# faverogian/diffusion-classifier

Measured on AMD Instinct MI355X. Metric: images classified/sec (node), CIFAR-10 10-class x 50-step ELBO scoring, higher is better.
Workload: dtype bf16; 1 GPU; cifar10-unet-10x50; classes=10, trials=50, forwards_per_image=500, input=uniform [-1,1], parallelism=single

## Files before the change

diffusion-classifier_amd/_lib.py:

```python
import ctypes as C
import os

_HERE = os.path.dirname(os.path.abspath(__file__))
LIB_PATH = os.environ.get("DCAMD_LIB") or os.path.join(_HERE, "libdcamd.so")

ABI_VERSION = 5
DC_F32, DC_BF16, DC_F16 = 0, 1, 2
ACT_NONE, ACT_SILU, ACT_GEGLU, ACT_GELU_TANH = 0, 1, 2, 3
OP_QSAMPLE, OP_SINUSOID, OP_IGEMM, OP_GROUPNORM, OP_LAYERNORM, OP_ATTENTION, OP_EPS_MSE, OP_TBLOCK_FRONT = 1, 2, 3, 4, 5, 6, 7, 8
OP_CROSS_ATTENTION = 9
OP_CROSS_ATTENTION_LEN = 10
OP_ATTENTION_BIAS, OP_RMSNORM, OP_EMBED_ROWS, OP_RELU = 11, 12, 13, 14
ATTENTION_BIAS_MAX_L = 512
OP_ATTENTION_CAUSAL, OP_LAYERNORM_ROWS, OP_EMBED_ROWS_POS, OP_ACT_PASS = 15, 16, 17, 18
ATTENTION_CAUSAL_MAX_L = 512
PASS_QUICK_GELU, PASS_GELU_ERF = 1, 2
OP_ERR_MAP = 19
EVIDENCE_FRAC_BITS, EVIDENCE_VMAX = 30, 16384.0
OP_ATTENTION_WIDE, OP_IM2COL_S2 = 20, 21
ATTENTION_WIDE_DIMS = (256, 512)

i32, i64, u64, f32, vp = C.c_int32, C.c_int64, C.c_uint64, C.c_float, C.c_void_p


class QsampleParams(C.Structure):
    _fields_ = [("x", vp), ("eps", vp), ("alpha", vp), ("sigma", vp), ("img_of_bj", vp),
                ("out", vp), ("out_dtype", i32),
                ("n_bj", i32), ("C", i32), ("H", i32), ("W", i32), ("ld", i32), ("im2col", i32), ("patch", i32)]


class SinusoidParams(C.Structure):
    _fields_ = [("lam", vp), ("out", vp), ("n", i32), ("dim", i32), ("flip_sin_to_cos", i32), ("freq_shift", f32)]


class IgemmParams(C.Structure):
    _fields_ = [("dtype", i32), ("taps", i32), ("stride", i32), ("upsample", i32),
                ("n_img", i32), ("Hin", i32), ("Win", i32), ("Hout", i32), ("Wout", i32),
                ("src0", vp), ("map0", vp), ("C0", i32), ("ld0", i32),
                ("src1", vp), ("map1", vp), ("C1", i32), ("ld1", i32),
                ("W", vp), ("Cout", i32), ("tile_n", i32),
                ("bias", vp),
                ("rowvec", vp), ("rowvec_map", vp), ("rowvec_ld", i32), ("act", i32),
                ("gate", vp), ("gate_map", vp), ("gate_ld", i32), ("pad2_", i32),
                ("residual", vp), ("res_map", vp), ("res_dtype", i32), ("res_ld", i32),
                ("out", vp), ("out_dtype", i32), ("out_ld", i32),
                ("gn_scale", vp), ("gn_shift", vp), ("gn_silu", i32), ("pad3_", i32),
                ("src2", vp), ("map2", vp), ("W2", vp), ("C2", i32), ("ld2", i32),
                ("ln_eps", f32), ("up4", i32), ("qstats", vp),
                ("pn_out", vp), ("pn_gamma", vp), ("pn_beta", vp), ("pn_cnt", vp),
                ("pn_ld", i32), ("pn_groups", i32), ("pn_silu", i32), ("pn_eps", f32)]


class GroupnormParams(C.Structure):
    _fields_ = [("x", vp), ("map0", vp), ("x1", vp), ("map1", vp),
                ("y", vp), ("dtype", i32), ("out_dtype", i32),
                ("n", i32), ("HW", i32), ("C", i32), ("C1", i32), ("groups", i32), ("silu", i32),
                ("splits", i32), ("eps", f32),
                ("gamma", vp), ("beta", vp), ("ws", vp), ("out_scale", vp), ("out_shift", vp),
                ("qstats", vp), ("qparts", i32), ("pad_", i32)]


class LayernormParams(C.Structure):
    _fields_ = [("x", vp), ("y", vp), ("dtype", i32), ("out_dtype", i32),
                ("rows", i32), ("C", i32), ("rows_per_sample", i32), ("mod_ld", i32), ("eps", f32),
                ("gamma", vp), ("beta", vp), ("scale", vp), ("shift", vp), ("mod_map", vp)]


class AttentionParams(C.Structure):
    _fields_ = [("q", vp), ("k", vp), ("v", vp), ("out", vp),
                ("dtype", i32), ("n", i32), ("L", i32), ("heads", i32), ("d", i32),
                ("ld_qkv", i32), ("ld_out", i32), ("scale", f32)]


class AttentionWideParams(C.Structure):
    _fields_ = AttentionParams._fields_


class Im2colS2Params(C.Structure):
    _fields_ = [("x", vp), ("out", vp), ("dtype", i32), ("n", i32), ("H", i32), ("W", i32), ("C", i32), ("ld", i32)]


class CrossAttentionParams(C.Structure):
    _fields_ = [("q", vp), ("k", vp), ("v", vp), ("out", vp), ("q_map", vp), ("kv_map", vp),
                ("dtype", i32), ("n", i32), ("Lq", i32), ("S", i32), ("heads", i32), ("d", i32),
                ("ld_q", i32), ("ld_kv", i32), ("ld_out", i32), ("scale", f32)]


class CrossAttentionLenParams(C.Structure):
    _fields_ = [("q", vp), ("k", vp), ("v", vp), ("out", vp), ("q_map", vp), ("kv_map", vp), ("kv_len", vp),
                ("dtype", i32), ("n", i32), ("Lq", i32), ("S", i32), ("heads", i32), ("d", i32),
                ("ld_q", i32), ("ld_kv", i32), ("ld_out", i32), ("scale", f32)]


class AttentionBiasParams(C.Structure):
    _fields_ = [("q", vp), ("k", vp), ("v", vp), ("out", vp), ("bias", vp), ("kv_len", vp),
                ("dtype", i32), ("n", i32), ("L", i32), ("heads", i32), ("d", i32), ("ld_qkv", i32), ("ld_out", i32), ("scale", f32)]


class RmsnormParams(C.Structure):
    _fields_ = [("x", vp), ("y", vp), ("weight", vp), ("row_len", vp),
                ("dtype", i32), ("out_dtype", i32), ("rows", i32), ("C", i32), ("rows_per_sample", i32), ("eps", f32)]


class EmbedRowsParams(C.Structure):
    _fields_ = [("table", vp), ("ids", vp), ("out", vp), ("out_dtype", i32), ("rows", i32), ("C", i32), ("vocab", i32)]


class ReluParams(C.Structure):
    _fields_ = [("x", vp), ("n", i64), ("dtype", i32), ("pad_", i32)]


class AttentionCausalParams(C.Structure):
    _fields_ = [("q", vp), ("k", vp), ("v", vp), ("out", vp), ("row_len", vp),
                ("dtype", i32), ("n", i32), ("L", i32), ("heads", i32), ("d", i32), ("ld_qkv", i32), ("ld_out", i32), ("scale", f32)]


class LayernormRowsParams(C.Structure):
    _fields_ = [("x", vp), ("y", vp), ("gamma", vp), ("beta", vp), ("row_len", vp),
                ("dtype", i32), ("out_dtype", i32), ("rows", i32), ("C", i32), ("rows_per_sample", i32), ("eps", f32)]


class EmbedRowsPosParams(C.Structure):
    _fields_ = [("table", vp), ("pos", vp), ("ids", vp), ("out", vp),
                ("out_dtype", i32), ("rows", i32), ("C", i32), ("vocab", i32), ("L", i32), ("pad_", i32)]


class ActPassParams(C.Structure):
    _fields_ = [("x", vp), ("n", i64), ("dtype", i32), ("kind", i32)]


class TblockFrontParams(C.Structure):
    _fields_ = [("x", vp), ("Wp", vp), ("bp", vp), ("ln_g", vp), ("ln_b", vp), ("Wqkv", vp), ("Wo", vp), ("bo", vp),
                ("rowvec", vp), ("rowvec_map", vp), ("out", vp),
                ("dtype", i32), ("n", i32), ("L", i32), ("C", i32), ("heads", i32), ("ldx", i32), ("ld_out", i32), ("rowvec_ld", i32),
                ("ln_eps", f32), ("scale", f32)]


class EpsMseParams(C.Structure):
    _fields_ = [("pred", vp), ("eps", vp), ("x", vp), ("alpha", vp), ("sigma", vp),
                ("bj_of_unit", vp), ("img_of_bj", vp), ("out_index", vp),
                ("out", vp), ("n_units", i32), ("C", i32), ("H", i32), ("W", i32), ("ld", i32), ("v_param", i32), ("patch", i32)]


class ErrMapParams(C.Structure):
    _fields_ = [("pred", vp), ("eps", vp), ("x", vp), ("alpha", vp), ("sigma", vp),
                ("bj_of_unit", vp), ("img_of_bj", vp), ("out_index", vp),
                ("acc", vp), ("bad", vp),
                ("n_units", i32), ("C", i32), ("H", i32), ("W", i32), ("ld", i32), ("v_param", i32), ("patch", i32),
                ("T", i32), ("cells", i32), ("pad_", i32)]


class EvidenceMapsParams(C.Structure):
    _fields_ = [("acc", vp), ("bad", vp), ("stage_ends", vp), ("n_eval", vp), ("winner", vp),
                ("mean_map", vp), ("delta_map", vp), ("invalid", vp),
                ("n_stages", i32), ("BS", i32), ("C", i32), ("HW", i32)]


class DdpmStepParams(C.Structure):
    _fields_ = [("z", vp), ("pred", vp), ("noise", vp), ("out", vp),
                ("n", i32), ("C", i32), ("H", i32), ("W", i32), ("ld", i32), ("patch", i32), ("v_param", i32),
                ("w", f32), ("alpha_t", f32), ("sigma_t", f32), ("alpha_s", f32), ("c", f32), ("sd", f32), ("one_plus_w", f32)]


class DdpmStepSharedParams(C.Structure):
    _fields_ = [("z", vp), ("pred", vp), ("noise", vp), ("out", vp),
                ("n", i32), ("C", i32), ("H", i32), ("W", i32), ("ld", i32), ("patch", i32), ("v_param", i32), ("noise_div", i32),
                ("w", f32), ("alpha_t", f32), ("sigma_t", f32), ("alpha_s", f32), ("c", f32), ("sd", f32), ("one_plus_w", f32), ("pad_", i32)]


class SolverStepParams(C.Structure):
    _fields_ = [("z", vp), ("pred", vp), ("xprev", vp), ("xhat", vp), ("out", vp),
                ("n", i32), ("C", i32), ("H", i32), ("W", i32), ("ld", i32), ("patch", i32), ("v_param", i32), ("clamp", i32), ("final_pass", i32),
                ("w", f32), ("one_plus_w", f32), ("alpha_t", f32), ("sigma_t", f32), ("k1", f32), ("k2", f32), ("k3", f32)]


class DdpmNoiseMapParams(C.Structure):
    _fields_ = [("z", vp), ("pred", vp), ("x_next", vp), ("out", vp),
                ("n", i32), ("C", i32), ("H", i32), ("W", i32), ("ld", i32), ("patch", i32), ("v_param", i32),
                ("w", f32), ("one_plus_w", f32), ("alpha_t", f32), ("sigma_t", f32), ("alpha_s", f32), ("c", f32), ("sd", f32)]


class AbsDiffMapParams(C.Structure):
    _fields_ = [("a", vp), ("r", vp), ("r_of_a", vp), ("out", vp),
                ("n", i32), ("m", i32), ("C", i32), ("H", i32), ("W", i32), ("pad_", i32)]


class ClassPosteriorParams(C.Structure):
    _fields_ = [("errors", vp), ("probs", vp), ("entropy", vp), ("margin", vp), ("margin_z", vp),
                ("winner", vp), ("runner", vp), ("invalid", vp), ("means", vp), ("delta", vp), ("n_eval", vp),
                ("BS", i32), ("C", i32), ("T", i32), ("t_end", i32), ("temperature", f32), ("pad_", i32)]


class Op(C.Structure):
    _fields_ = [("kind", i32), ("pad_", i32), ("params", vp)]


EXPORTS = ["dc_abi_version", "dc_last_error", "dc_arch", "dc_qsample", "dc_philox_normal", "dc_sinusoid",
           "dc_igemm", "dc_igemm_cout_pad", "dc_igemm_variant", "dc_igemm_instance", "dc_igemm_gn_fusable", "dc_igemm_side_ok", "dc_igemm_ln_ok", "dc_igemm_qstats_parts", "dc_igemm_up4_ok", "dc_igemm_pn_ok", "dc_pn_timeouts", "dc_groupnorm", "dc_groupnorm_variant", "dc_groupnorm_ws_floats", "dc_groupnorm_splits",
           "dc_layernorm", "dc_layernorm_variant", "dc_attention", "dc_attention_variant", "dc_attention_wide", "dc_attention_wide_variant", "dc_im2col_s2", "dc_cross_attention", "dc_cross_attention_variant", "dc_cross_attention_len", "dc_cross_attention_len_variant", "dc_attention_bias", "dc_attention_bias_variant", "dc_rmsnorm", "dc_embed_rows", "dc_relu", "dc_attention_causal", "dc_attention_causal_variant", "dc_layernorm_rows", "dc_embed_rows_pos", "dc_act_pass", "dc_tblock_front", "dc_tblock_front_ok", "dc_eps_mse", "dc_err_map", "dc_evidence_maps", "dc_ddpm_step", "dc_ddpm_step_shared", "dc_solver_step", "dc_ddpm_noise_map", "dc_abs_diff_map", "dc_haar_dwt2", "dc_haar_idwt2", "dc_stage_topk", "dc_reduce_argmin", "dc_stage_maps", "dc_stage_maps_rows", "dc_stage_stop", "dc_class_posterior", "dc_run_plan", "dc_run_plan_timed",
           "dc_packed_bytes", "dc_pack_weights_matrix", "dc_pack_weights_conv3x3", "dc_pack_weights_up4", "dc_pack_weights_geglu",
           "dc_fold_layernorm_bias", "dc_workspace_bytes_groupnorm", "dc_workspace_bytes_igemm", "dc_workspace_bytes_attention",
           "dc_workspace_bytes_layernorm"]

_lib = None


class DcamdError(RuntimeError):
    pass


def lib():
    global _lib
    if _lib is not None:
        return _lib
    if not os.path.exists(LIB_PATH):
        raise DcamdError(
            f"HIP extension {LIB_PATH} is missing — build it with `python -c 'import __graft_entry__ as g; g.build()'` "
            "(or `make -C diffusion-classifier_amd/csrc`). There is no CPU fallback for the scoring path.")
    L = C.CDLL(LIB_PATH)
    L.dc_abi_version.restype = i32
    L.dc_last_error.restype = C.c_char_p
    L.dc_arch.restype = C.c_char_p
    for name, argt in [("dc_qsample", [C.POINTER(QsampleParams), vp]),
                       ("dc_sinusoid", [C.POINTER(SinusoidParams), vp]),
                       ("dc_igemm", [C.POINTER(IgemmParams), vp]),
                       ("dc_groupnorm", [C.POINTER(GroupnormParams), vp]),
                       ("dc_layernorm", [C.POINTER(LayernormParams), vp]),
                       ("dc_attention", [C.POINTER(AttentionParams), vp]),
                       ("dc_attention_wide", [C.POINTER(AttentionWideParams), vp]),
                       ("dc_im2col_s2", [C.POINTER(Im2colS2Params), vp]),
                       ("dc_cross_attention", [C.POINTER(CrossAttentionParams), vp]),
                       ("dc_cross_attention_len", [C.POINTER(CrossAttentionLenParams), vp]),
                       ("dc_attention_bias", [C.POINTER(AttentionBiasParams), vp]),
                       ("dc_rmsnorm", [C.POINTER(RmsnormParams), vp]),
                       ("dc_embed_rows", [C.POINTER(EmbedRowsParams), vp]),
                       ("dc_relu", [C.POINTER(ReluParams), vp]),
                       ("dc_attention_causal", [C.POINTER(AttentionCausalParams), vp]),
                       ("dc_layernorm_rows", [C.POINTER(LayernormRowsParams), vp]),
                       ("dc_embed_rows_pos", [C.POINTER(EmbedRowsPosParams), vp]),
                       ("dc_act_pass", [C.POINTER(ActPassParams), vp]),
                       ("dc_tblock_front", [C.POINTER(TblockFrontParams), vp]),
                       ("dc_eps_mse", [C.POINTER(EpsMseParams), vp]),
                       ("dc_err_map", [C.POINTER(ErrMapParams), vp]),
                       ("dc_evidence_maps", [C.POINTER(EvidenceMapsParams), vp]),
                       ("dc_class_posterior", [C.POINTER(ClassPosteriorParams), vp]),
                       ("dc_ddpm_step", [C.POINTER(DdpmStepParams), vp]),
                       ("dc_ddpm_step_shared", [C.POINTER(DdpmStepSharedParams), vp]),
                       ("dc_solver_step", [C.POINTER(SolverStepParams), vp]),
                       ("dc_ddpm_noise_map", [C.POINTER(DdpmNoiseMapParams), vp]),
                       ("dc_abs_diff_map", [C.POINTER(AbsDiffMapParams), vp]),
                       ("dc_run_plan", [C.POINTER(Op), i32, vp]),
                       ("dc_run_plan_timed", [C.POINTER(Op), i32, vp, vp]),
                       ("dc_philox_normal", [vp, i64, i64, vp, u64, vp]),
                       ("dc_haar_dwt2", [vp, vp, i32, i32, i32, i32, f32, vp]),
                       ("dc_haar_idwt2", [vp, vp, i32, i32, i32, i32, f32, vp]),
                       ("dc_pack_weights_matrix", [vp, i32, i32, i32, vp, vp, vp, i32, i32, vp]),
                       ("dc_pack_weights_conv3x3", [vp, i32, i32, i32, i32, i32, vp, i32, i32, vp]),
                       ("dc_pack_weights_up4", [vp, i32, i32, vp, i32, i32, vp]),
                       ("dc_pack_weights_geglu", [vp, vp, i32, i32, vp, vp, vp, vp, vp, i32, vp]),
                       ("dc_fold_layernorm_bias", [vp, vp, vp, i32, i32, vp, vp]),
                       ("dc_stage_topk", [vp, i32, i32, i32, i32, i32, vp, vp, vp]),
                       ("dc_reduce_argmin", [vp, i32, i32, i32, i32, vp, vp, vp]),
                       ("dc_stage_maps", [vp, i32, i32, i32, i32, i32, i32, i32, i32, i32, i32, i32, vp, vp]),
                       ("dc_stage_maps_rows", [vp, vp, i32, i32, i32, i32, i32, i32, i32, i32, i32, i32, i32, i32, vp, vp]),
                       ("dc_stage_stop", [vp, i32, i32, i32, i32, f32, vp, vp, vp, vp, vp, vp])]:
        fn = getattr(L, name)
        fn.argtypes = argt
        fn.restype = i32
    L.dc_igemm_ln_ok.argtypes = [C.POINTER(IgemmParams)]
    L.dc_igemm_ln_ok.restype = C.c_int32
    L.dc_igemm_qstats_parts.argtypes = [C.POINTER(IgemmParams)]
    L.dc_igemm_qstats_parts.restype = C.c_int32
    L.dc_igemm_up4_ok.argtypes = [C.POINTER(IgemmParams)]
    L.dc_igemm_up4_ok.restype = C.c_int32
    L.dc_igemm_pn_ok.argtypes = [C.POINTER(IgemmParams)]
    L.dc_igemm_pn_ok.restype = C.c_int32
    L.dc_tblock_front_ok.argtypes = [C.POINTER(TblockFrontParams)]
    L.dc_tblock_front_ok.restype = C.c_int32
    L.dc_pn_timeouts.argtypes = []
    L.dc_pn_timeouts.restype = C.c_int32
    L.dc_igemm_side_ok.argtypes = [C.POINTER(IgemmParams)]
    L.dc_igemm_side_ok.restype = C.c_int32
    L.dc_igemm_variant.argtypes = [C.POINTER(IgemmParams)]
    L.dc_igemm_variant.restype = C.c_char_p
    L.dc_igemm_instance.argtypes = [C.POINTER(IgemmParams), C.POINTER(C.c_int32)]
    L.dc_igemm_instance.restype = C.c_char_p
    L.dc_attention_variant.argtypes = [C.POINTER(AttentionParams)]
    L.dc_attention_variant.restype = C.c_char_p
    L.dc_attention_wide_variant.argtypes = [C.POINTER(AttentionWideParams)]
    L.dc_attention_wide_variant.restype = C.c_char_p
    L.dc_cross_attention_variant.argtypes = [C.POINTER(CrossAttentionParams)]
    L.dc_cross_attention_variant.restype = C.c_char_p
    L.dc_cross_attention_len_variant.argtypes = [C.POINTER(CrossAttentionLenParams)]
    L.dc_cross_attention_len_variant.restype = C.c_char_p
    L.dc_attention_bias_variant.argtypes = [C.POINTER(AttentionBiasParams)]
    L.dc_attention_bias_variant.restype = C.c_char_p
    L.dc_attention_causal_variant.argtypes = [C.POINTER(AttentionCausalParams)]
    L.dc_attention_causal_variant.restype = C.c_char_p
    L.dc_groupnorm_variant.argtypes = [C.POINTER(GroupnormParams)]
    L.dc_groupnorm_variant.restype = C.c_char_p
    L.dc_layernorm_variant.argtypes = [C.POINTER(LayernormParams)]
    L.dc_layernorm_variant.restype = C.c_char_p
    L.dc_igemm_gn_fusable.argtypes = [C.POINTER(IgemmParams)]
    L.dc_igemm_gn_fusable.restype = i32
    L.dc_igemm_cout_pad.argtypes = [i32, i32]
    L.dc_igemm_cout_pad.restype = i32
    L.dc_packed_bytes.argtypes = [i32, i32, i32, i32]
    L.dc_packed_bytes.restype = i64
    for name, pt in (("dc_workspace_bytes_groupnorm", GroupnormParams), ("dc_workspace_bytes_igemm", IgemmParams),
                     ("dc_workspace_bytes_attention", AttentionParams), ("dc_workspace_bytes_layernorm", LayernormParams)):
        getattr(L, name).argtypes = [C.POINTER(pt)]
        getattr(L, name).restype = i64
    L.dc_groupnorm_ws_floats.argtypes = [i32, i32, i32]
    L.dc_groupnorm_ws_floats.restype = i64
    L.dc_groupnorm_splits.argtypes = [i32, i32, i32]
    L.dc_groupnorm_splits.restype = i32
    if L.dc_abi_version() != ABI_VERSION:
        raise DcamdError(f"libdcamd ABI {L.dc_abi_version()} != {ABI_VERSION} (stale libdcamd.so? rebuild with `make -C diffusion-classifier_amd/csrc`)")
    _lib = L
    return L


def check(rc, what=""):
    if rc != 0:
        raise DcamdError(f"{what} failed (status {rc}): {lib().dc_last_error().decode()}")


def stream_ptr():
    import torch
    return C.c_void_p(torch.cuda.current_stream().cuda_stream)


def require_gpu():
    import torch
    if not torch.cuda.is_available():
        raise DcamdError("the diffusion-classifier scoring path needs an MI355X (HIP device); no CPU fallback exists")
    return lib()
```

diffusion-classifier_amd/csrc/api.hip:

```cpp
#include <stdarg.h>
#include <stdio.h>
#include "common.h"

static thread_local char g_err[512] = "";

void dc_set_error(const char* fmt, ...) {
  va_list ap;
  va_start(ap, fmt);
  vsnprintf(g_err, sizeof(g_err), fmt, ap);
  va_end(ap);
}

int dc_check_launch(const char* what) {
  const hipError_t e = hipGetLastError();
  if (e != hipSuccess) {
    dc_set_error("%s: HIP launch failed: %s", what, hipGetErrorString(e));
    return DC_ERR_LAUNCH;
  }
  return DC_OK;
}

extern "C" int dc_abi_version(void) { return DC_ABI_VERSION; }
extern "C" const char* dc_last_error(void) { return g_err; }
extern "C" const char* dc_arch(void) { return "gfx950"; }

static int run_one(const dc_op* ops, int i, dc_stream s);

extern "C" int dc_run_plan(const dc_op* ops, int32_t n, dc_stream s) {
  DC_REQUIRE(ops || n == 0, DC_ERR_ARG, "dc_run_plan: null ops");
  for (int i = 0; i < n; ++i) {
    const int rc = run_one(ops, i, s);
    if (rc != DC_OK) return rc;
  }
  return DC_OK;
}

extern "C" int dc_run_plan_timed(const dc_op* ops, int32_t n, dc_stream s, float* ms) {
  DC_REQUIRE((ops && ms) || n == 0, DC_ERR_ARG, "dc_run_plan_timed: null ops/ms");
  hipStream_t st = reinterpret_cast<hipStream_t>(s);
  hipEvent_t* ev = new hipEvent_t[n + 1];
  for (int i = 0; i <= n; ++i) (void)hipEventCreate(&ev[i]);
  int rc = DC_OK;
  (void)hipEventRecord(ev[0], st);
  int done = 0;
  for (; done < n; ++done) {
    rc = run_one(ops, done, s);
    if (rc != DC_OK) break;
    (void)hipEventRecord(ev[done + 1], st);
  }
  (void)hipStreamSynchronize(st);
  for (int i = 0; i < done; ++i) (void)hipEventElapsedTime(&ms[i], ev[i], ev[i + 1]);
  for (int i = 0; i <= n; ++i) (void)hipEventDestroy(ev[i]);
  delete[] ev;
  return rc;
}

static int run_one(const dc_op* ops, int i, dc_stream s) {
  {
    int rc;
    switch (ops[i].kind) {
      case DC_OP_QSAMPLE: rc = dc_qsample(static_cast<const dc_qsample_params*>(ops[i].params), s); break;
      case DC_OP_SINUSOID: rc = dc_sinusoid(static_cast<const dc_sinusoid_params*>(ops[i].params), s); break;
      case DC_OP_IGEMM: rc = dc_igemm(static_cast<const dc_igemm_params*>(ops[i].params), s); break;
      case DC_OP_GROUPNORM: rc = dc_groupnorm(static_cast<const dc_groupnorm_params*>(ops[i].params), s); break;
      case DC_OP_LAYERNORM: rc = dc_layernorm(static_cast<const dc_layernorm_params*>(ops[i].params), s); break;
      case DC_OP_ATTENTION: rc = dc_attention(static_cast<const dc_attention_params*>(ops[i].params), s); break;
      case DC_OP_CROSS_ATTENTION: rc = dc_cross_attention(static_cast<const dc_cross_attention_params*>(ops[i].params), s); break;
      case DC_OP_CROSS_ATTENTION_LEN: rc = dc_cross_attention_len(static_cast<const dc_cross_attention_len_params*>(ops[i].params), s); break;
      case DC_OP_ATTENTION_BIAS: rc = dc_attention_bias(static_cast<const dc_attention_bias_params*>(ops[i].params), s); break;
      case DC_OP_RMSNORM: rc = dc_rmsnorm(static_cast<const dc_rmsnorm_params*>(ops[i].params), s); break;
      case DC_OP_EMBED_ROWS: rc = dc_embed_rows(static_cast<const dc_embed_rows_params*>(ops[i].params), s); break;
      case DC_OP_RELU: rc = dc_relu(static_cast<const dc_relu_params*>(ops[i].params), s); break;
      case DC_OP_ATTENTION_CAUSAL: rc = dc_attention_causal(static_cast<const dc_attention_causal_params*>(ops[i].params), s); break;
      case DC_OP_LAYERNORM_ROWS: rc = dc_layernorm_rows(static_cast<const dc_layernorm_rows_params*>(ops[i].params), s); break;
      case DC_OP_EMBED_ROWS_POS: rc = dc_embed_rows_pos(static_cast<const dc_embed_rows_pos_params*>(ops[i].params), s); break;
      case DC_OP_ACT_PASS: rc = dc_act_pass(static_cast<const dc_act_pass_params*>(ops[i].params), s); break;
      case DC_OP_TBLOCK_FRONT: rc = dc_tblock_front(static_cast<const dc_tblock_front_params*>(ops[i].params), s); break;
      case DC_OP_EPS_MSE: rc = dc_eps_mse(static_cast<const dc_eps_mse_params*>(ops[i].params), s); break;
      case DC_OP_ERR_MAP: rc = dc_err_map(static_cast<const dc_err_map_params*>(ops[i].params), s); break;
      case DC_OP_ATTENTION_WIDE: rc = dc_attention_wide(static_cast<const dc_attention_wide_params*>(ops[i].params), s); break;
      case DC_OP_IM2COL_S2: rc = dc_im2col_s2(static_cast<const dc_im2col_s2_params*>(ops[i].params), s); break;
      default: dc_set_error("dc_run_plan: op %d has unknown kind %d", i, ops[i].kind); return DC_ERR_ARG;
    }
    if (rc != DC_OK) {
      char inner[400];
      snprintf(inner, sizeof(inner), "%s", g_err);
      dc_set_error("dc_run_plan: op %d (kind %d) failed: %s", i, ops[i].kind, inner);
      return rc;
    }
  }
  return DC_OK;
}
```

diffusion-classifier_amd/csrc/conv3_halo.h:

```cpp
#pragma once
#include <stdlib.h>
#include "igemm_epilogue.h"

typedef const __attribute__((address_space(1))) void* gptr_t;
typedef __attribute__((address_space(3))) void* lptr_t;

struct HaloGeom {
  int ltw, lth, lni;
  int tiles_x, tiles_y;
  int hw, hp, HR, nxl;
  int n_img, H, W;
  float inv_hp, inv_hw;
  int mos, lmc;
  float inv_ch, inv_cw;
  int xbuf;
  int sws;
  int lpt;
};


constexpr int HALO_WST = 128 * 64;

inline int dc_conv3_halo_waves(int H, int W) { return (H <= 8 || W <= 8) ? 8 : 4; }

template <int NW> struct HaloCfg {
  static constexpr int NT = NW * 64;
  static constexpr int PIX = NW * 64;
  static constexpr int NXL = NW == 4 ? 6 : 7;
  static constexpr int XBUF = NXL * NT * 16;
  static constexpr int XROWS = NXL * NT / 4;
  static constexpr int WLD = 512 / NT;
  static constexpr int WR = NW == 4 ? 3 : 4;
  static constexpr int GNOFF = 2 * XBUF + WR * HALO_WST;
  static constexpr int GNMAXC = 512;
  static constexpr int TBLOFF = GNOFF + 2 * GNMAXC * 4;
  static constexpr int LDS_MAIN = TBLOFF + 128;
  static constexpr int LDS = LDS_MAIN;
};

__device__ __forceinline__ int swz64(int row) { return (0x78 >> (((row >> 2) & 3) << 1)) & 3; }
__device__ __forceinline__ int lds64_off(int row, int chunk) { return row * 64 + ((chunk ^ swz64(row)) << 4); }


struct HaloQs {
  static constexpr bool on = true;
  int nbase, ltp, n_img, tile_in_img, wm, np, padd;
  __device__ __forceinline__ bool whole() const { return ltp >= 7; }
  __device__ __forceinline__ int parts() const { return np; }
  __device__ __forceinline__ bool operator()(int half, int& n, int& part) const {
    const int p0 = wm * 128 + half * 64;
    n = nbase + (p0 >> ltp);
    part = padd + (ltp >= 7 ? (tile_in_img << (ltp - 7)) + ((p0 & ((1 << ltp) - 1)) >> 7) : tile_in_img);
    return n < n_img;
  }
};

struct HaloLdsBias {
  static constexpr bool on = true, has_rowvec = true;
  const float* p;
  __device__ __forceinline__ void operator()(int k, float (&bs)[8], float (&)[8]) const {
    const f32x4 lo = *reinterpret_cast<const f32x4*>(p + 32 * k), hi = *reinterpret_cast<const f32x4*>(p + 32 * k + 4);
#pragma unroll
    for (int e = 0; e < 4; ++e) { bs[e] = lo[e]; bs[4 + e] = hi[e]; }
  }
};

template <int N> __device__ __forceinline__ void hwait_vmcnt() { asm volatile("s_waitcnt vmcnt(%0)" ::"n"(N) : "memory"); }

template <int V> struct IC { static constexpr int value = V; };

#ifndef HALO_XDEPTH
#define HALO_XDEPTH 3
#endif
```

diffusion-classifier_amd/csrc/conv3_halo.hip:

```cpp
#include <stdlib.h>
#include "common.h"
#ifdef DC_STAMPS
static __device__ unsigned long long* g_stamps;
extern "C" void dc_debug_set_stamps(unsigned long long* p) { (void)hipMemcpyToSymbol(HIP_SYMBOL(g_stamps), &p, sizeof(p)); }
#define DC_STAMP(k) do { if (threadIdx.x == 0 && g_stamps) g_stamps[blockIdx.x * 8 + (k)] = __builtin_amdgcn_s_memtime(); } while (0)
static __device__ int g_halo_abl;
extern "C" void dc_debug_set_halo_abl(int v) { (void)hipMemcpyToSymbol(HIP_SYMBOL(g_halo_abl), &v, sizeof(v)); }
#define DC_HALO_ABL() __builtin_amdgcn_readfirstlane(g_halo_abl)
#else
#define DC_STAMP(k) do {} while (0)
#define DC_HALO_ABL() 0
#endif
#include "igemm_epilogue.h"
#include "epi_pn.h"

static __device__ unsigned g_pn_timeouts;
static __device__ chunk16 g_zero_page[16];
#include "conv3_halo_plan.h"
DC_CLOCK_DECL(conv3_halo)

template <typename T, int NW, int NTAP = 9, int MODE = 0, bool STG = false, bool PN = false>
__global__ __launch_bounds__(NW * 64, 2) void conv3_halo_kernel(const IgemmArgs a, const HaloGeom g) {
  static_assert(!PN || (MODE == 1 && NW == 4 && !STG) || ((MODE == 0 || MODE == 2) && NW == 8 && STG && NTAP == 9), "producer-side GroupNorm: one-image-per-patch forms, or 8x8 / 4x4 images");
  constexpr bool PNX = PN && NW == 4, PNL = PN && NW == 8;
  static_assert(!STG || NW == 8, "staggered loop: the 8-wave kernel");
  constexpr bool XB = MODE == 1, MOS = MODE == 2;
  using Cfg = HaloCfg<NW>;
  constexpr int EPC = Elem<T>::EPC;
  constexpr int BKE = 4 * EPC;
  constexpr int TM = 8, TN = 4;
  constexpr int NT = Cfg::NT, WLD = Cfg::WLD, WR = Cfg::WR, PD = Cfg::WR - 1;
  extern __shared__ __attribute__((aligned(16))) char smem[];
  char* const Wring = smem + 2 * Cfg::XBUF;

  DC_STAMP(0);
  const int t = threadIdx.x;
  const int lane = t & 63;
  const int wave = __builtin_amdgcn_readfirstlane(t >> 6);
  const int wm = wave >> 1, wn = wave & 1;
  const int lr = lane & 15, lq = lane >> 4;
  int tile_m, tile_n;
  if constexpr (PNX) {
    constexpr int LPH = NTAP == 4 ? 2 : 0;
    const int tnr = a.tiles_n >> LPH;
    const int kq = blockIdx.x >> 3;
    const int grp = ((kq >> (g.lpt + LPH)) << 3) + (blockIdx.x & 7);
    if (grp >= g.n_img * tnr) return;
    const int smp = grp / tnr;
    const int within = kq & ((1 << (g.lpt + LPH)) - 1);
    tile_n = __builtin_amdgcn_readfirstlane((within >> g.lpt) * tnr + grp - smp * tnr);
    tile_m = __builtin_amdgcn_readfirstlane((smp << g.lpt) + (within & ((1 << g.lpt) - 1)));
    asm volatile("" : "+s"(tile_m), "+s"(tile_n));
  } else if constexpr (XB) tile_of_block_scalar(a, tile_m, tile_n);
  else tile_of_block(a, tile_m, tile_n);
  constexpr bool UP4 = NTAP == 4;
  int phase = 0;
  if (UP4) { const int tn = a.tiles_n >> 2; phase = tile_n / tn; tile_n -= phase * tn; }
  const int pa = phase >> 1, pb = phase & 1;
  int tx = tile_m % g.tiles_x;
  int ty = (tile_m / g.tiles_x) % g.tiles_y;
  int ng = tile_m / (g.tiles_x * g.tiles_y);
  const int tw = 1 << g.ltw, th = 1 << g.lth;
  const int HW = g.H * g.W;
  const int HWs = a.upsample ? (g.H >> 1) * (g.W >> 1) : HW;
  const int Ctot = a.C0 + a.C1;
  const int c0chunks = a.C0 / BKE, nchunks = Ctot / BKE;

  constexpr int NXL = Cfg::NXL;
  int pp[NXL];
  const int xlx = t & 3;
  int* const tbl = reinterpret_cast<int*>(smem + Cfg::TBLOFF);
  if (t < (1 << g.lni)) {
    const int n = (ng << g.lni) + t;
    const bool vn = n < g.n_img;
    tbl[4 * t] = vn ? (a.map0 ? a.map0[n] : n) * HWs : -1;
    tbl[4 * t + 1] = (vn && a.src1) ? (a.map1 ? a.map1[n] : n) * HWs : -1;
    tbl[4 * t + 2] = (vn && a.src2) ? (a.map2 ? a.map2[n] : n) * HWs : -1;
  }
  auto piece_code = [&](int i, int* col = nullptr) -> int {
    const int hr = (i * NT + t) >> 2;
    int code = -1;
    if (col) *col = 0;
    if (i < g.nxl && hr < g.HR) {
      if constexpr (MOS) {
        const int hy = (int)(((float)hr + 0.5f) * g.inv_hw), hx = hr - hy * g.hw;
        const int cy = (int)(((float)hy + 0.5f) * g.inv_ch), ry = hy - cy * (th + 1);
        const int cx = (int)(((float)hx + 0.5f) * g.inv_cw), rx = hx - cx * (tw + 1);
        if (col) *col = hx;
        if (ry > 0 && rx > 0) code = (((cy << g.lmc) + cx) << 20) | ((ry - 1) * g.W + rx - 1);
      } else {
        const int img = (int)(((float)hr + 0.5f) * g.inv_hp), r = hr - img * g.hp;
        const int hy = (int)(((float)r + 0.5f) * g.inv_hw), hx = r - hy * g.hw;
        const int iy = ty * th + hy - 1, ix = tx * tw + hx - 1;
        if (col) *col = hx;
        if ((unsigned)iy < (unsigned)g.H && (unsigned)ix < (unsigned)g.W)
          code = (img << 20) | (a.upsample ? (iy >> 1) * (g.W >> 1) + (ix >> 1) : iy * g.W + ix);
      }
    }
    return code;
  };
  constexpr bool SWP = !STG;
#pragma unroll
  for (int i = 0; i < NXL; ++i) {
    int col;
    pp[i] = piece_code(i, &col);
// ... 299 lines not shown
  DC_CLOCK(0);
  for (int cc = 0; cc < nchunks; ++cc) {
    const bool side_next = cc + 1 == nchunks && nx > 0;
    const bool has_next = cc + 1 < nchunks || side_next;
    const int s0 = cc * NTAP;
    const uint32_t xbo = (uint32_t)(cc & 1) * Cfg::XBUF;
    auto step = [&](auto tapc) {
      constexpr int tap = decltype(tapc)::value;
      if (has_next) {
        if (tap >= 1 && tap <= PD) hwait_vmcnt<FLYL + NXL>();
        else hwait_vmcnt<FLYL>();
      } else {
        constexpr int left = NTAP - 1 - tap;
        hwait_vmcnt<(left < PD - 1 ? left : PD - 1) * WLD>();
      }
      __builtin_amdgcn_s_barrier();
      constexpr int t2 = tap + PD;
      if (t2 < NTAP) issue_w(cc, t2, (s0 + t2) % WR);
      else if (side_next) { if (t2 - NTAP < nx) issue_w2(t2 - NTAP, (s0 + t2) % WR); }
      else if (has_next) issue_w(cc + 1, t2 - NTAP, (s0 + t2) % WR);
      if (tap == 0 && has_next) issue_x(cc + 1);

      const uint32_t wso = (uint32_t)((s0 + tap) % WR) * HALO_WST;
      constexpr int ky = UP4 ? (tap >> 1) : tap / 3, kx = UP4 ? (tap & 1) : tap - ky * 3;
      const int tapoff = ((ky + pa) * g.hw + kx + pb) * 64;
      mma_tap(wso, xbo, tapoff, IC<kx>{});
    };
    step(IC<0>{}); step(IC<1>{}); step(IC<2>{}); step(IC<3>{});
    if constexpr (NTAP == 9) { step(IC<4>{}); step(IC<5>{}); step(IC<6>{}); step(IC<7>{}); step(IC<8>{}); }
  }

  DC_CLOCK(1);
  }
  constexpr int FLY = (PD - 1) * WLD;
  {
    const int NSm = nchunks * NTAP;
    for (int e = 0; e < nx; ++e) {
      if (e == 0 && nx >= PD) hwait_vmcnt<FLY>();
      else hwait_vmcnt<0>();
      __builtin_amdgcn_s_barrier();
      if (e + PD < nx) issue_w2(e + PD, (NSm + e + PD) % WR);
      if (e + 1 < nx) issue_x(nchunks + e + 1);
      const uint32_t xbo = (uint32_t)((nchunks + e) & 1) * Cfg::XBUF;
      const uint32_t wso = (uint32_t)((NSm + e) % WR) * HALO_WST;
      const int tapoff = (g.hw + 1) * 64;
      mma_tap(wso, xbo, tapoff, IC<1>{});
    }
  }

  DC_STAMP(2);
  if constexpr (!XB) asm volatile("" : "+v"(tx), "+v"(ty), "+v"(ng), "+v"(tile_n));
  const int nw0 = min((ng << g.lni) + ((wm * 128) >> (g.ltw + g.lth)), g.n_img - 1);
  const int nw1 = min((ng << g.lni) + ((wm * 128 + 127) >> (g.ltw + g.lth)), g.n_img - 1);
  HaloQs qsfn;
  qsfn.nbase = ng << g.lni; qsfn.ltp = g.ltw + g.lth; qsfn.n_img = g.n_img; qsfn.tile_in_img = ty * g.tiles_x + tx; qsfn.wm = wm;
  qsfn.np = HW >= 128 ? HW >> 7 : 1;
  qsfn.padd = 0;
  if (UP4) { qsfn.padd = phase * qsfn.np; qsfn.np *= 4; }
  auto rowfn = [&](int j, EpiRow& r) {
    const int p = wm * 128 + j * 16 + lr;
    int n = (ng << g.lni) + (p >> (g.ltw + g.lth));
    r.ok = n < g.n_img;
    n = r.ok ? n : g.n_img - 1;
    const int py = (p >> g.ltw) & (th - 1), px = p & (tw - 1);
    const int rem = (ty * th + py) * g.W + tx * tw + px;
    r.samp = n;
    r.o = UP4 ? n * (4 * HW) + (2 * (ty * th + py) + pa) * (2 * g.W) + 2 * (tx * tw + px) + pb : n * HW + rem;
    r.r = (a.residual && a.res_map ? a.res_map[n] : n) * HW + rem;
  };
  if constexpr (PNL && MOS) {
    epi_direct_act<T, TM, DC_ACT_NONE, false, false>(a, acc, tile_n, wn, lq, nw0, nw1, rowfn, EpiNoPre(), qsfn, EpiNoBias(), EpiPnLocal4x4());
  } else if constexpr (PNL) {
    epi_direct_act<T, TM, DC_ACT_NONE, false, true>(a, acc, tile_n, wn, lq, nw0, nw1, rowfn, EpiNoPre(), qsfn, EpiNoBias(), EpiPnLocal8x8());
  } else if constexpr (PNX) {
    PnCtx pc;
    pc.sample = ng; pc.part = (UP4 ? phase * (HW >> 7) : 0) + ((ty * g.tiles_x + tx) << 1) + wm;
    pc.parts = (HW >> 7) << (UP4 ? 2 : 0); pc.tiles = 1 << (g.lpt + (UP4 ? 2 : 0));
    pc.qpg = (a.Cout / a.pn_groups) >> 2;
    pc.cnt = a.pn_cnt + (size_t)ng * (UP4 ? a.tiles_n >> 2 : a.tiles_n) + tile_n; pc.timeouts = &g_pn_timeouts;
    pc.gam = brv + 128 + wn * 64 + lq * 8; pc.bet = brv + 256 + wn * 64 + lq * 8;
    pc.scr = reinterpret_cast<float2*>(pc.tiles > 1 ? smem + wave * 4096 : smem + wn * 256);
    pc.flag = reinterpret_cast<int*>(brv + 384);
    pc.eps = a.pn_eps; pc.silu = a.pn_silu;
    epi_halo_pn<T>(a, acc, tile_n, wn, lq, rowfn, brv + wn * 64 + lq * 8, pc);
  } else if constexpr (STAGE_BRV) {
    epi_direct_act<T, TM, DC_ACT_NONE, false, true>(a, acc, tile_n, wn, lq, nw0, nw1, rowfn, EpiNoPre(), qsfn, HaloLdsBias{brv + wn * 64 + lq * 8});
  } else {
    epi_direct_act<T, TM, DC_ACT_NONE, false, !MOS>(a, acc, tile_n, wn, lq, nw0, nw1, rowfn, EpiNoPre(), qsfn);
  }
  DC_STAMP(7);
}

struct ThinCfg {
  static constexpr int NT = 256, NXL = 6;
  static constexpr int XBUF = NXL * NT * 16;
  static constexpr int WBUF = 3 * NT * 16;
  static constexpr int TBLOFF = 2 * XBUF + 2 * WBUF;
  static constexpr int LDS = TBLOFF + 128;
  static constexpr int GNOFF = LDS, GNMAXC = 512;
  static constexpr int LDS_GN = GNOFF + 2 * GNMAXC * 4;
};

template <typename T, bool GN>
__global__ __launch_bounds__(256, 2) void conv3_thin_kernel(const IgemmArgs a, const HaloGeom g) {
  using Cfg = ThinCfg;
  constexpr int EPC = Elem<T>::EPC;
  constexpr int BKE = 4 * EPC;
  constexpr int TM = 4, NT = Cfg::NT, NXL = Cfg::NXL;
  extern __shared__ __attribute__((aligned(16))) char smem[];
  char* const Wl = smem + 2 * Cfg::XBUF;
  const int t = threadIdx.x;
  const int lane = t & 63;
  const int wave = __builtin_amdgcn_readfirstlane(t >> 6);
  const int lr = lane & 15, lq = lane >> 4;
  const int tile_m = blockIdx.x;
  const int tx = tile_m % g.tiles_x;
  const int ty = (tile_m / g.tiles_x) % g.tiles_y;
  const int ng = tile_m / (g.tiles_x * g.tiles_y);
  const int tw = 1 << g.ltw, th = 1 << g.lth;
  const int HW = g.H * g.W;
  const int Ctot = a.C0 + a.C1;
  const int c0chunks = a.C0 / BKE, nchunks = Ctot / BKE;

  int pp[NXL];
  const int xlx = t & 3;
  int* const tbl = reinterpret_cast<int*>(smem + Cfg::TBLOFF);
  if (t < (1 << g.lni)) {
    const int n = (ng << g.lni) + t;
    const bool vn = n < g.n_img;
    tbl[4 * t] = vn ? (a.map0 ? a.map0[n] : n) * HW : -1;
    tbl[4 * t + 1] = (vn && a.src1) ? (a.map1 ? a.map1[n] : n) * HW : -1;
  }
#pragma unroll
  for (int i = 0; i < NXL; ++i) {
    const int hr = (i * NT + t) >> 2;
    pp[i] = -1;
    if (i < g.nxl && hr < g.HR) {
      const int img = (int)(((float)hr + 0.5f) * g.inv_hp), r = hr - img * g.hp;
      const int hy = (int)(((float)r + 0.5f) * g.inv_hw), hx = r - hy * g.hw;
      const int iy = ty * th + hy - 1, ix = tx * tw + hx - 1;
      if ((unsigned)iy < (unsigned)g.H && (unsigned)ix < (unsigned)g.W) pp[i] = (img << 20) | (iy * g.W + ix);
    }
  }
  __syncthreads();
  const char* zero = reinterpret_cast<const char*>(g_zero_page);
  auto issue = [&](int cc) {
    const int which = cc >= c0chunks ? 1 : 0;
    const T* src = reinterpret_cast<const T*>(which ? a.src1 : a.src0);
    const int ld = which ? a.ld1 : a.ld0;
    const int coff = (which ? cc - c0chunks : cc) * BKE + xlx * EPC;
    char* xs = smem + (cc & 1) * Cfg::XBUF + wave * 1024;
#pragma unroll
    for (int i = 0; i < NXL; ++i) {
      int pk = pp[i];
      asm volatile("" : "+v"(pk));
      const int base = pk < 0 ? -1 : tbl[4 * (pk >> 20) + which];
      const size_t e = (size_t)(base < 0 ? 0 : base + (pk & 0xFFFFF)) * ld + coff;
      const char* gp = base < 0 ? zero : reinterpret_cast<const char*>(src + e);
      __builtin_amdgcn_global_load_lds((gptr_t)gp, (lptr_t)(xs + i * (NT * 16)), 16, 0, 0);
    }
    char* ws = Wl + (cc & 1) * Cfg::WBUF + wave * 1024;
#pragma unroll
    for (int i = 0; i < 3; ++i) {
      const int p = i * NT + t;
      const int tap = p >> 6, row = (p >> 2) & 15;
      const bool ok = tap < 9;
// ... 128 lines not shown
  HaloKey& k = pl.key;
  k = HaloKey{NW, up4 ? 4 : 9, 0, false, false};
  const bool fits = halo_geom(g, a.Hin, a.Win, n_img, NW * 64, NW * 64, NW == 4 ? HaloCfg<4>::NXL : HaloCfg<8>::NXL, NW == 8);
  const int ni = 1 << g.lni;
  if ((g.H < 8 || g.W < 8) && !g.mos) return halo_plan_fail(pl, "conv3_halo: %dx%d images need the 8-wave patch", g.H, g.W);
  g.sws = (g.ltw < 4 ? g.ltw : 4) - 2;
  const long long es = dc_dtype_size(dtype);
  g.xbuf = (ni == 1 && !g.mos && halo_xbuf_reach(a, dtype)) ? 1 : 0;
  k.MODE = g.mos ? 2 : (g.xbuf ? 1 : 0);
  if ((long long)a.tiles_n * 128 * a.Ktot >= (1LL << 31)) return halo_plan_fail(pl, "conv3_halo: weight matrix of %d x %d too large", a.tiles_n * 128, a.Ktot);
  if (!fits || g.nxl < 3) return halo_plan_fail(pl, "conv3_halo: halo of %d rows does not fit", g.HR);
  pl.tiles_m = ((n_img + ni - 1) / ni) * g.tiles_x * g.tiles_y;
  long long grid = (long long)pl.tiles_m * a.tiles_n;
  if (grid <= 0 || grid > 0x7fffffffLL) return halo_plan_fail(pl, "conv3_halo: bad grid %lld", grid);
  k.STG = NW == 8 && !up4 && !getenv("DCAMD_HALO_NO_STAG") && (long long)a.tiles_n * 128 * a.Ktot * es < (1LL << 31);
  if (a.pn_out) {
    if (NW == 4) {
      if (!g.xbuf || ni != 1) return halo_plan_fail(pl, "conv3_halo: producer-side GroupNorm needs the one-image-per-patch form");
      const long long groups = (long long)n_img * (up4 ? a.tiles_n >> 2 : a.tiles_n);
      grid = ((groups + 7) / 8 * 8) << (g.lpt + (up4 ? 2 : 0));
      if (grid > 0x7fffffffLL) return halo_plan_fail(pl, "conv3_halo: bad grid %lld", grid);
    } else {
      const bool i8 = !g.mos && !g.xbuf && g.H == 8 && g.W == 8 && ni == 8, i4 = g.mos && g.H == 4 && g.W == 4 && ni == 32;
      if (up4 || !(i8 || i4)) return halo_plan_fail(pl, "conv3_halo: producer-side GroupNorm on the 8-wave patch needs 8x8 or 4x4 images");
      if (!k.STG) return halo_plan_fail(pl, "conv3_halo: producer-side GroupNorm on 8x8 images needs the staggered loop");
    }
    k.PN = true;
  }
  pl.grid = (unsigned)grid;
  return pl;
}

using HaloKern = void (*)(const IgemmArgs, const HaloGeom);

template <typename T, int NW, int NTAP, int MODE, bool STG = false, bool PN = false>
static HaloKern halo_instance() {
  static bool attr_done = false;
  const HaloKern kern = conv3_halo_kernel<T, NW, NTAP, MODE, STG, PN>;
  if (!attr_done) {
    (void)hipFuncSetAttribute(reinterpret_cast<const void*>(kern), hipFuncAttributeMaxDynamicSharedMemorySize, HaloCfg<NW>::LDS);
    attr_done = true;
  }
  return kern;
}

template <typename T>
static HaloKern halo_kernel(const HaloKey& k) {
  auto is = [&](int nw, int ntap, int mode, bool stg = false, bool pn = false) {
    return k.NW == nw && k.NTAP == ntap && k.MODE == mode && k.STG == stg && k.PN == pn;
  };
  if (is(8, 4, 0)) return halo_instance<T, 8, 4, 0>();
  if (is(8, 9, 0)) return halo_instance<T, 8, 9, 0>();
  if (is(8, 9, 1)) return halo_instance<T, 8, 9, 1>();
  if (is(8, 4, 1)) return halo_instance<T, 8, 4, 1>();
  if (is(8, 9, 2)) return halo_instance<T, 8, 9, 2>();
  if (is(8, 4, 2)) return halo_instance<T, 8, 4, 2>();
  if (is(8, 9, 2, true, true)) return halo_instance<T, 8, 9, 2, true, true>();
  if (is(8, 9, 0, true, true)) return halo_instance<T, 8, 9, 0, true, true>();
  if (is(8, 9, 0, true)) return halo_instance<T, 8, 9, 0, true>();
  if (is(8, 9, 1, true)) return halo_instance<T, 8, 9, 1, true>();
  if (is(8, 9, 2, true)) return halo_instance<T, 8, 9, 2, true>();
  if (is(4, 4, 0)) return halo_instance<T, 4, 4, 0>();
  if (is(4, 9, 0)) return halo_instance<T, 4, 9, 0>();
  if (is(4, 9, 1)) return halo_instance<T, 4, 9, 1>();
  if (is(4, 4, 1)) return halo_instance<T, 4, 4, 1>();
  if (is(4, 4, 1, false, true)) return halo_instance<T, 4, 4, 1, false, true>();
  if (is(4, 9, 1, false, true)) return halo_instance<T, 4, 9, 1, false, true>();
  return nullptr;
}

int dc_conv3_halo_launch(const HaloPlan& pl, const IgemmArgs& a0, int dtype, bool up4, hipStream_t s) {
  if (pl.status != DC_OK) { dc_set_error("%s", pl.message); return pl.status; }
  IgemmArgs a = up4 ? dc_conv3_up4_walked(a0) : a0;
  a.tiles_m = pl.tiles_m;
  const HaloKey& k = pl.key;
  HaloKern kern = nullptr;
  const int rc = dc_by_dtype(dtype, "dc_igemm: dtype", [&](auto t) { kern = halo_kernel<decltype(t)>(k); return (int)DC_OK; });
  if (rc != DC_OK) return rc;
  if (!kern) { dc_set_error("conv3_halo: no instance <%d,%d,%d,%d,%d>", k.NW, k.NTAP, k.MODE, (int)k.STG, (int)k.PN); return DC_ERR_UNSUPPORTED; }
  hipLaunchKernelGGL(kern, dim3(pl.grid), dim3(k.NW * 64), k.NW == 4 ? HaloCfg<4>::LDS : HaloCfg<8>::LDS, s, a, pl.g);
  return dc_check_launch("dc_igemm(conv3_halo)");
}

constexpr int PN_MAX_TILES = 16;
bool dc_conv3_halo_pn_ok(const IgemmArgs& a, const HaloPlan& pl, bool up4) {
  static const bool off = getenv("DCAMD_NO_PN") != nullptr;
  if (off || a.src1 || (!up4 && a.upsample)) return false;
  if (pl.status != DC_OK || !pl.key.PN) return false;
  if (((1 << pl.g.lpt) << (up4 ? 2 : 0)) > PN_MAX_TILES) return false;
  if (a.Cout % 128 || a.pn_groups <= 0 || a.Cout % a.pn_groups) return false;
  const int cpg = a.Cout / a.pn_groups;
  return cpg == 4 || cpg == 8 || cpg == 16 || cpg == 32;
}

unsigned dc_conv3_halo_pn_timeouts() {
  unsigned v = 0, z = 0;
  if (hipMemcpyFromSymbol(&v, HIP_SYMBOL(g_pn_timeouts), sizeof(v)) != hipSuccess) return ~0u;
  if (v) (void)hipMemcpyToSymbol(HIP_SYMBOL(g_pn_timeouts), &z, sizeof(z));
  return v;
}

HaloPlan dc_conv3_thin_plan(const IgemmArgs& a, int n_img) {
  HaloPlan pl;
  pl.key = HaloKey{4, 9, 0, false, false};
  HaloGeom& g = pl.g;
  if (!halo_geom(g, a.Hin, a.Win, n_img, 256, ThinCfg::NT, ThinCfg::NXL, false)) return halo_plan_fail(pl, "conv3_thin: halo of %d rows does not fit", g.HR);
  const int ni = 1 << g.lni;
  const long long nblk = (long long)((n_img + ni - 1) / ni) * g.tiles_x * g.tiles_y;
  if (nblk <= 0 || nblk > 0x7fffffffLL) return halo_plan_fail(pl, "conv3_thin: bad grid %lld", nblk);
  if (a.gn_scale && ni != 1) return halo_plan_fail(pl, "conv3_thin: the fused GroupNorm needs one sample per patch");
  pl.tiles_m = (int)nblk; pl.grid = (unsigned)nblk;
  return pl;
}

template <typename T>
static int launch_thin(const HaloPlan& pl, const IgemmArgs& a, hipStream_t s) {
  static bool attr_done = false;
  const bool gn = a.gn_scale != nullptr;
  void (*kern)(const IgemmArgs, const HaloGeom) = gn ? conv3_thin_kernel<T, true> : conv3_thin_kernel<T, false>;
  const int lds = gn ? ThinCfg::LDS_GN : ThinCfg::LDS;
  if (!attr_done) {
    (void)hipFuncSetAttribute(reinterpret_cast<const void*>(conv3_thin_kernel<T, false>), hipFuncAttributeMaxDynamicSharedMemorySize, ThinCfg::LDS);
    (void)hipFuncSetAttribute(reinterpret_cast<const void*>(conv3_thin_kernel<T, true>), hipFuncAttributeMaxDynamicSharedMemorySize, ThinCfg::LDS_GN);
    attr_done = true;
  }
  hipLaunchKernelGGL(kern, dim3(pl.grid), dim3(ThinCfg::NT), lds, s, a, pl.g);
  return dc_check_launch("dc_igemm(conv3_thin)");
}

int dc_conv3_thin_launch(const IgemmArgs& a, int dtype, int n_img, hipStream_t s) {
  const HaloPlan pl = dc_conv3_thin_plan(a, n_img);
  if (pl.status != DC_OK) { dc_set_error("%s", pl.message); return pl.status; }
  return dc_by_dtype(dtype, "dc_igemm: dtype", [&](auto t) { return launch_thin<decltype(t)>(pl, a, s); });
}
```

diffusion-classifier_amd/csrc/conv3_halo_plan.h:

```cpp
#pragma once
#include <stdarg.h>
#include <stdio.h>
#include "conv3_halo.h"

static inline int ilog2(int v) { int l = 0; while ((1 << l) < v) ++l; return l; }

static inline bool halo_geom(HaloGeom& g, int H, int W, int n_img, int pix, int nt, int nxl_cap, bool mosaic_ok) {
  g.H = H; g.W = W; g.n_img = n_img;
  const int tw = W < 32 ? W : 32;
  int th = pix / tw; if (th > H) th = H;
  const int ni = pix / (tw * th);
  g.ltw = ilog2(tw); g.lth = ilog2(th); g.lni = ilog2(ni);
  g.tiles_x = W / tw; g.tiles_y = H / th;
  g.hw = tw + 2; g.hp = (th + 2) * g.hw; g.HR = ni * g.hp;
  g.mos = 0; g.lmc = 0; g.inv_ch = g.inv_cw = 0.f;
  if (mosaic_ok && (H < 8 || W < 8) && tw == W && th == H && ni >= 2) {
    g.mos = 1;
    g.lmc = (g.lni + 1) / 2;
    const int cols = 1 << g.lmc, rows = ni >> g.lmc;
    g.hw = cols * (tw + 1) + 1;
    g.hp = 0;
    g.HR = (rows * (th + 1) + 1) * g.hw;
    g.inv_ch = 1.0f / (float)(th + 1); g.inv_cw = 1.0f / (float)(tw + 1);
  }
  g.inv_hp = g.hp ? 1.0f / (float)g.hp : 0.f; g.inv_hw = 1.0f / (float)g.hw;
  g.xbuf = 0; g.sws = 0;
  g.lpt = ilog2(g.tiles_x * g.tiles_y);
  g.nxl = (g.HR * 4 + nt - 1) / nt;
  return g.nxl <= nxl_cap;
}

static inline bool halo_xbuf_reach(const IgemmArgs& a, int dtype) {
  const long long es = dc_dtype_size(dtype);
  const long long hws = (long long)(a.upsample ? (a.Hin >> 1) * (a.Win >> 1) : a.Hin * a.Win);
  const long long ldmax = a.ld0 > a.ld1 ? (a.ld0 > a.ld2 ? a.ld0 : a.ld2) : (a.ld1 > a.ld2 ? a.ld1 : a.ld2);
  return hws * ldmax * es < (1LL << 31) && (long long)a.tiles_n * 128 * a.Ktot * es < (1LL << 31);
}

struct HaloKey { int NW, NTAP, MODE; bool STG, PN; };

struct HaloPlan {
  HaloGeom g;
  int tiles_m = 0;
  unsigned grid = 0;
  HaloKey key{};
  int status = DC_OK;
  char message[112] = "";
};

__attribute__((format(printf, 2, 3))) static inline HaloPlan& halo_plan_fail(HaloPlan& pl, const char* fmt, ...) {
  pl.status = DC_ERR_SHAPE;
  va_list ap;
  va_start(ap, fmt);
  vsnprintf(pl.message, sizeof(pl.message), fmt, ap);
  va_end(ap);
  return pl;
}

static inline void halo_plan_ints(const HaloPlan& pl, int32_t* out) {
  const HaloGeom& g = pl.g;
  const int32_t v[14] = {1 << g.ltw, 1 << g.lth, 1 << g.lni, g.tiles_x, g.tiles_y, g.hw, g.HR, g.nxl, g.mos, g.xbuf, g.sws, g.lpt, pl.tiles_m, (int32_t)pl.grid};
  for (int i = 0; i < 14; ++i) out[i] = v[i];
}

HaloPlan dc_conv3_halo_plan(const IgemmArgs& walked, int dtype, int n_img, bool up4);
int dc_conv3_halo_launch(const HaloPlan& pl, const IgemmArgs& a, int dtype, bool up4, hipStream_t s);
bool dc_conv3_halo_pn_ok(const IgemmArgs& a, const HaloPlan& pl, bool up4);
HaloPlan dc_conv3_thin_plan(const IgemmArgs& a, int n_img);
HaloPlan dc_conv3_ws_plan(const IgemmArgs& a, int n_img);
```

diffusion-classifier_amd/csrc/elementwise.hip:

```cpp
#include "common.h"

struct QsArgs {
  const float* x; const float* eps; const float* alpha; const float* sigma; const int32_t* img_of_bj;
  void* out; int out_dtype, n_bj, C, H, W, ld, im2col, patch;
};

template <typename TO>
__global__ __launch_bounds__(256) void qsample_kernel(const QsArgs a) {
  constexpr int EPC = Elem<TO>::EPC;
  const int cpr = a.ld / EPC;
  const int HW = a.H * a.W;
  const int pp = a.im2col == 2 ? a.patch : 1;
  const int gw = a.W / pp, rows_per = (a.H / pp) * gw;
  const long long total = (long long)a.n_bj * rows_per * cpr;
  for (long long idx = blockIdx.x * 256LL + threadIdx.x; idx < total; idx += (long long)gridDim.x * 256) {
    const int ch = (int)(idx % cpr);
    const long long row = idx / cpr;
    const int p = (int)(row % rows_per);
    const int bj = (int)(row / rows_per);
    const int img = a.img_of_bj ? a.img_of_bj[bj] : bj;
    const float al = a.alpha[bj], sg = a.sigma[bj];
    const int y = p / gw, xw = p - y * gw;
    float f[EPC];
#pragma unroll
// ... 446 lines not shown
      t[2 * j] = (a[j] + hh[j] + v[j] + d[j]) * k;  t[2 * j + 1] = (a[j] + hh[j] - v[j] - d[j]) * k;
      b[2 * j] = (a[j] - hh[j] + v[j] - d[j]) * k;  b[2 * j + 1] = (a[j] - hh[j] - v[j] + d[j]) * k;
    }
    float* dst = out + (r * 2 * h + 2 * y) * (long long)(2 * w) + 8 * xq;
    __builtin_nontemporal_store(hv4_make(t[0], t[1], t[2], t[3]), reinterpret_cast<hv4*>(dst));
    __builtin_nontemporal_store(hv4_make(t[4], t[5], t[6], t[7]), reinterpret_cast<hv4*>(dst) + 1);
    __builtin_nontemporal_store(hv4_make(b[0], b[1], b[2], b[3]), reinterpret_cast<hv4*>(dst + 2 * w));
    __builtin_nontemporal_store(hv4_make(b[4], b[5], b[6], b[7]), reinterpret_cast<hv4*>(dst + 2 * w) + 1);
  }
}

static unsigned haar_grid(long long items) {
  const long long b = (items + 255) / 256;
  return (unsigned)(b > 65536 ? 65536 : b);
}

extern "C" int dc_haar_dwt2(const float* in, float* out, int32_t n, int32_t C, int32_t H, int32_t W, float scale, dc_stream stream) {
  DC_REQUIRE(in && out && n > 0 && C > 0 && H > 0 && W > 0, DC_ERR_ARG, "dc_haar_dwt2: bad args");
  DC_REQUIRE(H % 2 == 0 && W % 2 == 0, DC_ERR_SHAPE, "dc_haar_dwt2: H=%d W=%d must be even", H, W);
  DC_REQUIRE(((uintptr_t)in & 7) == 0, DC_ERR_ALIGN, "dc_haar_dwt2: input must be 8-byte aligned");
  const long long total = (long long)n * C * (H / 2) * (W / 2);
  if (W % 8 == 0 && (((uintptr_t)in | (uintptr_t)out) & 15) == 0) {
    hipLaunchKernelGGL(haar_dwt2_v4_kernel, dim3(haar_grid(total / 4)), dim3(256), 0, reinterpret_cast<hipStream_t>(stream), in, out,
                       total / 4, C, H, W, scale);
    return dc_check_launch("dc_haar_dwt2");
  }
  const unsigned grid = (unsigned)((total + 255) / 256 > 16384 ? 16384 : (total + 255) / 256);
  hipLaunchKernelGGL(haar_dwt2_kernel, dim3(grid), dim3(256), 0, reinterpret_cast<hipStream_t>(stream), in, out, total, C, H, W, scale);
  return dc_check_launch("dc_haar_dwt2");
}
extern "C" int dc_haar_idwt2(const float* in, float* out, int32_t n, int32_t C, int32_t h, int32_t w, float scale, dc_stream stream) {
  DC_REQUIRE(in && out && n > 0 && C > 0 && h > 0 && w > 0, DC_ERR_ARG, "dc_haar_idwt2: bad args");
  DC_REQUIRE(((uintptr_t)out & 7) == 0, DC_ERR_ALIGN, "dc_haar_idwt2: output must be 8-byte aligned");
  const long long total = (long long)n * C * h * w;
  if (w % 4 == 0 && (((uintptr_t)in | (uintptr_t)out) & 15) == 0) {
    hipLaunchKernelGGL(haar_idwt2_v4_kernel, dim3(haar_grid(total / 4)), dim3(256), 0, reinterpret_cast<hipStream_t>(stream), in, out,
                       total / 4, C, h, w, scale);
    return dc_check_launch("dc_haar_idwt2");
  }
  const unsigned grid = (unsigned)((total + 255) / 256 > 16384 ? 16384 : (total + 255) / 256);
  hipLaunchKernelGGL(haar_idwt2_kernel, dim3(grid), dim3(256), 0, reinterpret_cast<hipStream_t>(stream), in, out, total, C, h, w, scale);
  return dc_check_launch("dc_haar_idwt2");
}

template <typename U>
__global__ __launch_bounds__(256) void im2col_s2_kernel(const U* __restrict__ x, U* __restrict__ out, long long total, int H, int W, int Cu, int ldu) {
  const int Ho = H / 2, Wo = W / 2;
  for (long long idx = blockIdx.x * 256LL + threadIdx.x; idx < total; idx += (long long)gridDim.x * 256) {
    const int c = (int)(idx % Cu); long long r = idx / Cu;
    const int tap = (int)(r % 9); r /= 9;
    const int ox = (int)(r % Wo); r /= Wo;
    const int oy = (int)(r % Ho);
    const long long i = r / Ho;
    const int iy = 2 * oy + tap / 3, ix = 2 * ox + tap % 3;
    U v = {};
    if (iy < H && ix < W) v = x[((i * H + iy) * W + ix) * ldu + c];
    out[idx] = v;
  }
}

extern "C" int dc_im2col_s2(const dc_im2col_s2_params* p, dc_stream stream) {
  DC_REQUIRE(p && p->x && p->out, DC_ERR_ARG, "dc_im2col_s2: null pointer");
  DC_REQUIRE(p->dtype == DC_F32 || p->dtype == DC_BF16 || p->dtype == DC_F16, DC_ERR_DTYPE, "dc_im2col_s2: dtype %d", p->dtype);
  DC_REQUIRE(p->n > 0 && p->C > 0 && p->H > 0 && p->W > 0, DC_ERR_SHAPE, "dc_im2col_s2: extents n=%d C=%d H=%d W=%d", p->n, p->C, p->H, p->W);
  DC_REQUIRE(p->H % 2 == 0 && p->W % 2 == 0, DC_ERR_SHAPE, "dc_im2col_s2: H=%d W=%d must be even", p->H, p->W);
  DC_REQUIRE(p->ld >= p->C, DC_ERR_SHAPE, "dc_im2col_s2: ld=%d < C=%d", p->ld, p->C);
  const int es = dc_dtype_size(p->dtype), epc = 16 / es;
  DC_REQUIRE((((uintptr_t)p->x | (uintptr_t)p->out) & (uintptr_t)(es - 1)) == 0, DC_ERR_ALIGN, "dc_im2col_s2: x/out must be element aligned");
  const long long elems = (long long)p->n * (p->H / 2) * (p->W / 2) * 9 * p->C;
  hipStream_t s = reinterpret_cast<hipStream_t>(stream);
  auto grid = [](long long items) { const long long b = (items + 255) / 256; return (unsigned)(b > 65536 ? 65536 : b); };
  if (p->C % epc == 0 && p->ld % epc == 0 && (((uintptr_t)p->x | (uintptr_t)p->out) & 15) == 0) {
    hipLaunchKernelGGL(im2col_s2_kernel<chunk16>, dim3(grid(elems / epc)), dim3(256), 0, s, reinterpret_cast<const chunk16*>(p->x),
                       reinterpret_cast<chunk16*>(p->out), elems / epc, p->H, p->W, p->C / epc, p->ld / epc);
  } else if (es == 4) {
    hipLaunchKernelGGL(im2col_s2_kernel<uint32_t>, dim3(grid(elems)), dim3(256), 0, s, reinterpret_cast<const uint32_t*>(p->x),
                       reinterpret_cast<uint32_t*>(p->out), elems, p->H, p->W, p->C, p->ld);
  } else {
    hipLaunchKernelGGL(im2col_s2_kernel<uint16_t>, dim3(grid(elems)), dim3(256), 0, s, reinterpret_cast<const uint16_t*>(p->x),
                       reinterpret_cast<uint16_t*>(p->out), elems, p->H, p->W, p->C, p->ld);
  }
  return dc_check_launch("dc_im2col_s2");
}
```

diffusion-classifier_amd/csrc/epi_pn.h:

```cpp
#pragma once
#include "igemm_epilogue.h"

#ifndef PN_TIMEOUT_TICKS
#define PN_TIMEOUT_TICKS 3000000ull
#endif

struct PnCtx {
  int sample;
  int part;
  int parts;
  int tiles;
  int qpg;
  unsigned* cnt;
  unsigned* timeouts;
  const float* gam;
  const float* bet;
  float2* scr;
  int* flag;
  float eps;
  int silu;
};

__device__ __forceinline__ void pn_fold_row(const float2* scr, int parts, int q0, int qpg, int lr, float nq, float& mean, float& var) {
#pragma clang fp contract(off)
  auto row_sum = [](float v) {
    v += __builtin_bit_cast(float, __builtin_amdgcn_update_dpp(0, __builtin_bit_cast(int, v), 0xB1, 0xF, 0xF, true));
    v += __builtin_bit_cast(float, __builtin_amdgcn_update_dpp(0, __builtin_bit_cast(int, v), 0x4E, 0xF, 0xF, true));
    v += __builtin_bit_cast(float, __builtin_amdgcn_update_dpp(0, __builtin_bit_cast(int, v), 0x141, 0xF, 0xF, true));
    v += __builtin_bit_cast(float, __builtin_amdgcn_update_dpp(0, __builtin_bit_cast(int, v), 0x140, 0xF, 0xF, true));
    return v;
  };
  const float piv = scr[q0].x;
  float s1 = 0.f, s2 = 0.f, s3 = 0.f;
  for (int p = lr; p < parts; p += 16)
    for (int q = q0; q < q0 + qpg; ++q) {
      const float2 v = scr[p * 16 + q];
      const float d = v.x - piv;
      s1 += d; s3 = __builtin_fmaf(d, d, s3); s2 += v.y;
    }
  s1 = row_sum(s1); s2 = row_sum(s2); s3 = row_sum(s3);
  const float R = (float)(parts * qpg), iR = 1.0f / R;
  mean = __builtin_fmaf(s1, iR, piv);
  const float m2 = __builtin_fmaf(nq, fmaxf(__builtin_fmaf(-s1 * s1, iR, s3), 0.f), s2);
  var = fmaxf(m2 / (R * nq), 0.f);
}

template <typename T, typename RowFn>
__device__ __forceinline__ void epi_halo_pn(const IgemmArgs& a, f32x4 (&acc)[4][8], int tile_n, int wn, int lq, RowFn rowfn,
                                            const float* brv, const PnCtx& c) {
  constexpr int TM = 8, NK = 2;
  constexpr bool res16 = sizeof(T) == 2;
  const int abl = DC_HALO_ABL();
  const int c0 = tile_n * 128 + wn * 64 + lq * 8;
#pragma unroll
  for (int k = 0; k < NK; ++k) {
    const f32x4 lo = *reinterpret_cast<const f32x4*>(brv + 32 * k), hi = *reinterpret_cast<const f32x4*>(brv + 32 * k + 4);
#pragma unroll
    for (int j = 0; j < TM; ++j) { acc[2 * k][j] += lo; acc[2 * k + 1][j] += hi; }
  }
  int orow[TM];
  {
    EpiRow row[TM];
#pragma unroll
    for (int j = 0; j < TM; ++j) { rowfn(j, row[j]); orow[j] = row[j].o; }
    if (a.residual) {
      if (res16) {
        chunk16 rc[TM][NK];
#pragma unroll
        for (int j = 0; j < TM; ++j)
#pragma unroll
          for (int k = 0; k < NK; ++k)
            rc[j][k] = *reinterpret_cast<const chunk16*>(reinterpret_cast<const char*>(a.residual) + ((size_t)row[j].r * a.res_ld + c0 + 32 * k) * 2);
#pragma unroll
        for (int j = 0; j < TM; ++j)
#pragma unroll
          for (int k = 0; k < NK; ++k) {
            float rf[8];
            chunk_to_f<T>(rc[j][k], rf);
#pragma unroll
            for (int e = 0; e < 8; ++e) acc[2 * k + (e >> 2)][j][e & 3] += rf[e];
          }
      } else {
#pragma unroll
        for (int j = 0; j < TM; ++j)
#pragma unroll
          for (int k = 0; k < NK; ++k) {
            float rf[8];
            ld8(reinterpret_cast<const float*>(a.residual) + (size_t)row[j].r * a.res_ld + c0 + 32 * k, rf);
#pragma unroll
            for (int e = 0; e < 8; ++e) acc[2 * k + (e >> 2)][j][e & 3] += rf[e];
          }
      }
    }
  }
  DC_STAMP(3);
  f32x4 rec;
  {
#pragma clang fp contract(off)
    typedef __attribute__((ext_vector_type(2))) float f32x2;
    auto share0 = [](float v) { return __builtin_bit_cast(float, __builtin_amdgcn_update_dpp(0, __builtin_bit_cast(int, v), 0x150, 0xF, 0xF, true)); };
    auto row_sum = [](float v) {
      v += __builtin_bit_cast(float, __builtin_amdgcn_update_dpp(0, __builtin_bit_cast(int, v), 0xB1, 0xF, 0xF, true));
      v += __builtin_bit_cast(float, __builtin_amdgcn_update_dpp(0, __builtin_bit_cast(int, v), 0x4E, 0xF, 0xF, true));
      v += __builtin_bit_cast(float, __builtin_amdgcn_update_dpp(0, __builtin_bit_cast(int, v), 0x141, 0xF, 0xF, true));
      v += __builtin_bit_cast(float, __builtin_amdgcn_update_dpp(0, __builtin_bit_cast(int, v), 0x140, 0xF, 0xF, true));
      return v;
    };
    float piv[NK][2];
    f32x2 sm[NK][2], sq[NK][2];
#pragma unroll
    for (int k = 0; k < NK; ++k)
#pragma unroll
      for (int qd = 0; qd < 2; ++qd) {
        piv[k][qd] = share0(acc[2 * k + qd][0][0]);
        sm[k][qd] = f32x2{0.f, 0.f}; sq[k][qd] = f32x2{0.f, 0.f};
      }
#pragma unroll
    for (int j = 0; j < TM; ++j)
#pragma unroll
      for (int k = 0; k < NK; ++k)
#pragma unroll
        for (int qd = 0; qd < 2; ++qd)
#pragma unroll
          for (int e = 0; e < 4; e += 2) {
            const f32x2 d = f32x2{acc[2 * k + qd][j][e], acc[2 * k + qd][j][e + 1]} - f32x2{piv[k][qd], piv[k][qd]};
            sm[k][qd] += d;
            sq[k][qd] = __builtin_elementwise_fma(d, d, sq[k][qd]);
          }
    const float inv_n = 1.0f / (float)(TM * 16 * 4);
    float r[NK][4];
#pragma unroll
    for (int k = 0; k < NK; ++k)
// ... 13 lines not shown
    if (a.out) {
      if (a.out_dtype == DC_F32) {
  #pragma unroll
        for (int j = 0; j < TM; ++j)
  #pragma unroll
          for (int k = 0; k < NK; ++k) {
            float* op = reinterpret_cast<float*>(a.out) + (size_t)orow[j] * a.out_ld + c0 + 32 * k;
            *reinterpret_cast<f32x4*>(op) = acc[2 * k][j]; *reinterpret_cast<f32x4*>(op + 4) = acc[2 * k + 1][j];
          }
      } else {
  #pragma unroll
        for (int j = 0; j < TM; ++j)
  #pragma unroll
          for (int k = 0; k < NK; ++k) {
            float v[8];
  #pragma unroll
            for (int e = 0; e < 8; ++e) v[e] = acc[2 * k + (e >> 2)][j][e & 3];
            *reinterpret_cast<chunk16*>(reinterpret_cast<T*>(a.out) + (size_t)orow[j] * a.out_ld + c0 + 32 * k) = f_to_chunk<T>(v);
          }
      }
    }
  };
  bool ok = true;
  if (c.tiles == 1) {
    if (lrp < 2) *reinterpret_cast<f32x4*>(grec) = rec;
    __syncthreads();
    DC_STAMP(4);
    if (lrp < 2) *reinterpret_cast<f32x4*>(c.scr + c.part * 16 + qpub) = rec;
    __syncthreads();
    DC_STAMP(5);
    store_raw();
  } else {
    if (lrp < 2) asm volatile("global_store_dwordx4 %0, %1, off sc1" ::"v"(grec), "v"(rec) : "memory");
    asm volatile("s_waitcnt vmcnt(0)" ::: "memory");
    __syncthreads();
    DC_STAMP(4);
    unsigned ticket = 0;
    if (threadIdx.x == 0) ticket = __hip_atomic_fetch_add(c.cnt, 1u, __ATOMIC_RELAXED, __HIP_MEMORY_SCOPE_AGENT);
    store_raw();
    if (threadIdx.x < 64) {
      ticket = __builtin_amdgcn_readfirstlane(ticket);
      const unsigned target = (ticket & ~(unsigned)(c.tiles - 1)) + (unsigned)c.tiles;
      const unsigned long long t0 = __builtin_amdgcn_s_memrealtime();
      ok = false;
      for (;;) {
        const unsigned seen = __builtin_amdgcn_readfirstlane(__hip_atomic_load(c.cnt, __ATOMIC_RELAXED, __HIP_MEMORY_SCOPE_AGENT));
        if ((int)(seen - target) >= 0 || (abl & 16)) { ok = true; break; }
        if (__builtin_amdgcn_s_memrealtime() - t0 > PN_TIMEOUT_TICKS) break;
        __builtin_amdgcn_s_sleep(4);
      }
      if (threadIdx.x == 0) {
        *c.flag = ok ? 1 : 0;
        if (!ok) __hip_atomic_fetch_add(c.timeouts, 1u, __ATOMIC_RELAXED, __HIP_MEMORY_SCOPE_AGENT);
      }
    }
    __syncthreads();
    ok = *c.flag != 0;
    DC_STAMP(5);
    {
      const int lane = threadIdx.x & 63;
      const int CQ = a.Cout >> 2;
      const float* recs = a.qstats + ((size_t)c.sample * c.parts * CQ + ((tile_n * 128 + wn * 64) >> 2)) * 2;
      const int npair = c.parts * 8;
      f32x4 v[4];
#pragma unroll
      for (int u = 0; u < 4; ++u) {
        const int i = lane + 64 * u;
        v[u] = f32x4{0.f, 0.f, 0.f, 0.f};
        if (i < npair) {
          const float* p = recs + ((size_t)(i >> 3) * CQ + 2 * (i & 7)) * 2;
          asm volatile("global_load_dwordx4 %0, %1, off sc1" : "=v"(v[u]) : "v"(p) : "memory");
        }
      }
      asm volatile("s_waitcnt vmcnt(0)" : "+v"(v[0]), "+v"(v[1]), "+v"(v[2]), "+v"(v[3])::"memory");
#pragma unroll
      for (int u = 0; u < 4; ++u) {
        const int i = lane + 64 * u;
        if (i < npair) *reinterpret_cast<f32x4*>(c.scr + 2 * i) = v[u];
      }
    }
  }
  __builtin_amdgcn_s_waitcnt(0xC07F);
  __builtin_amdgcn_wave_barrier();
  float ga[NK][8], gb[NK][8];
  {
    const float nq = 512.0f;
    const int lr = threadIdx.x & 15;
#pragma unroll
    for (int k = 0; k < NK; ++k) {
      const int ql = 2 * lq + 8 * k;
      float mean[2], rstd[2];
      if (c.qpg == 1) {
#pragma unroll
        for (int h = 0; h < 2; ++h) {
          float var;
          pn_fold_row(c.scr, c.parts, ql + h, 1, lr, nq, mean[h], var);
          rstd[h] = rsqrtf(var + c.eps);
        }
      } else {
        float var;
        pn_fold_row(c.scr, c.parts, (ql / c.qpg) * c.qpg, c.qpg, lr, nq, mean[0], var);
        mean[1] = mean[0]; rstd[0] = rstd[1] = rsqrtf(var + c.eps);
      }
      if (!ok) rstd[0] = rstd[1] = __builtin_nanf("");
      float gm[8], bt[8];
      ld8(c.gam + 32 * k, gm);
      ld8(c.bet + 32 * k, bt);
#pragma unroll
      for (int e = 0; e < 8; ++e) {
        const float s = rstd[e >> 2] * gm[e];
        ga[k][e] = s; gb[k][e] = bt[e] - mean[e >> 2] * s;
      }
    }
  }
  DC_STAMP(6);
  auto store_norm = [&](auto actc) {
    constexpr bool ACT = decltype(actc)::value;
#pragma unroll
    for (int j = 0; j < TM; ++j)
#pragma unroll
      for (int k = 0; k < NK; ++k) {
        float v[8];
#pragma unroll
        for (int e = 0; e < 8; ++e) {
          float x = acc[2 * k + (e >> 2)][j][e & 3] * ga[k][e] + gb[k][e];
          if (ACT) x = silu_t<T>(x);
          v[e] = x;
        }
        T* op = reinterpret_cast<T*>(a.pn_out) + (size_t)orow[j] * a.pn_ld + c0 + 32 * k;
        if constexpr (sizeof(T) == 4) {
          *reinterpret_cast<f32x4*>(op) = f32x4{v[0], v[1], v[2], v[3]};
          *reinterpret_cast<f32x4*>(reinterpret_cast<float*>(op) + 4) = f32x4{v[4], v[5], v[6], v[7]};
        } else {
          *reinterpret_cast<chunk16*>(op) = f_to_chunk<T>(v);
        }
      }
  };
  if (c.silu && !(abl & 32)) store_norm(EpiIC<1>{});
  else store_norm(EpiIC<0>{});
}
```

diffusion-classifier_amd/csrc/igemm.hip:

```cpp
#include <stdio.h>
#include <stdlib.h>
#include "conv3_halo_plan.h"

template <typename T, int BM, int BN, int WGM, int WGN>
__global__ __launch_bounds__(256, 2) void igemm_kernel(const IgemmArgs a) {
  constexpr int EPC = Elem<T>::EPC;
  constexpr int BKE = 8 * EPC;
  constexpr int XL = BM / 32;
  constexpr int WL = (BN + 31) / 32;
  constexpr int WTM = BM / WGM, WTN = BN / WGN;
  constexpr int TM = WTM / 16, TN = WTN / 16;
  static_assert(WGM * WGN == 4, "4 waves");
  extern __shared__ __attribute__((aligned(16))) char smem[];
  constexpr int BUF = (BM + BN) * 128;

  const int t = threadIdx.x;
  const int lane = t & 63, wave = t >> 6;
  const int wm = wave / WGN, wn = wave % WGN;
  const int lr = lane & 15, lq = lane >> 4;

  int tile_m, tile_n;
  tile_of_block(a, tile_m, tile_n);

  const int HWo = a.Hout * a.Wout;
// ... 291 lines not shown
extern "C" int dc_igemm(const dc_igemm_params* p, dc_stream stream) {
  IgemmArgs a;
  const int rc = igemm_validate_and_fill(p, a);
  if (rc != DC_OK) return rc;
  const IgemmChoice c = igemm_choose(p, a);
  if (c.status != DC_OK) { dc_set_error("%s", c.message); return c.status; }
  return igemm_launch(c, a, p, stream);
}

extern "C" const char* dc_igemm_variant(const dc_igemm_params* p) {
  IgemmArgs a;
  if (igemm_validate_and_fill(p, a) != DC_OK) return "invalid";
  const IgemmChoice c = igemm_choose(p, a);
  return c.status == DC_OK ? igemm_name(c, p->dtype) : c.tag;
}

extern "C" const char* dc_igemm_instance(const dc_igemm_params* p, int32_t* geom) {
  IgemmArgs a;
  if (igemm_validate_and_fill(p, a) != DC_OK) return "invalid";
  const IgemmChoice c = igemm_choose(p, a);
  if (c.status != DC_OK) return c.tag;
  static thread_local char name[64];
  const char* dn = p->dtype == DC_BF16 ? "bf16" : (p->dtype == DC_F16 ? "f16" : "f32");
  HaloPlan pl;
  switch (c.kernel) {
    case IG_HALO: case IG_UP4_HALO: {
      pl = c.halo;
      const HaloKey& k = pl.key;
      snprintf(name, sizeof(name), "conv3_halo_kernel<%s,%d,%d,%d%s%s>", dn, k.NW, k.NTAP, k.MODE, k.STG ? ",stag" : "", k.PN ? ",pn" : "");
      break;
    }
    case IG_THIN: pl = dc_conv3_thin_plan(a, p->n_img); snprintf(name, sizeof(name), "conv3_thin_kernel<%s,%s>", dn, a.gn_scale ? "gn" : "plain"); break;
    case IG_WS: pl = dc_conv3_ws_plan(a, p->n_img); snprintf(name, sizeof(name), "conv3_ws_kernel<%s,%s>", dn, a.gn_scale ? "gn" : "plain"); break;
    default: return igemm_name(c, p->dtype);
  }
  if (geom) halo_plan_ints(pl, geom);
  return name;
}

static int32_t igemm_accepts(const dc_igemm_params& q) {
  IgemmArgs a;
  return igemm_validate_and_fill(&q, a) == DC_OK && igemm_choose(&q, a).status == DC_OK ? 1 : 0;
}
alignas(16) static float g_probe_dummy[4] = {0.f, 0.f, 0.f, 0.f};

extern "C" int32_t dc_igemm_gn_fusable(const dc_igemm_params* p) {
  if (!p) return 0;
  dc_igemm_params q = *p;
  q.gn_scale = g_probe_dummy; q.gn_shift = g_probe_dummy;
  return igemm_accepts(q);
}

extern "C" int32_t dc_igemm_ln_ok(const dc_igemm_params* p) {
  if (!p) return 0;
  dc_igemm_params q = *p;
  if (!(q.ln_eps > 0.f)) q.ln_eps = 1e-5f;
  return igemm_accepts(q);
}

extern "C" int32_t dc_igemm_qstats_parts(const dc_igemm_params* p) {
  if (!p) return 0;
  dc_igemm_params q = *p;
  if (!q.qstats) q.qstats = g_probe_dummy;
  if (!igemm_accepts(q)) return 0;
  const int hw = p->Hout * p->Wout;
  if (p->up4) { const int lo = hw >> 2; return 4 * (lo >= 128 ? lo / 128 : 1); }
  return hw >= 128 ? hw / 128 : 1;
}

extern "C" int32_t dc_igemm_pn_ok(const dc_igemm_params* p) {
  if (!p || p->pn_groups <= 0) return 0;
  dc_igemm_params q = *p;
  if (!q.pn_out) q.pn_out = g_probe_dummy;
  if (!q.qstats && !(q.Hin == 4 && q.Win == 4)) q.qstats = g_probe_dummy;
  if (!q.pn_gamma) q.pn_gamma = g_probe_dummy;
  if (!q.pn_beta) q.pn_beta = g_probe_dummy;
  if (!q.pn_cnt) q.pn_cnt = reinterpret_cast<uint32_t*>(g_probe_dummy);
  if (!(q.pn_eps > 0.f)) q.pn_eps = 1e-5f;
  return igemm_accepts(q);
}

extern "C" int32_t dc_pn_timeouts(void) { return (int32_t)dc_conv3_halo_pn_timeouts(); }

extern "C" int32_t dc_igemm_up4_ok(const dc_igemm_params* p) {
  if (!p) return 0;
  dc_igemm_params q = *p;
  q.up4 = 1;
  return igemm_accepts(q);
}

extern "C" int32_t dc_igemm_side_ok(const dc_igemm_params* p) {
  if (!p) return 0;
  dc_igemm_params q = *p;
  if (!q.src2) { q.src2 = g_probe_dummy; q.W2 = g_probe_dummy; }
  return igemm_accepts(q);
}
```

diffusion-classifier_amd/engine.py:

```python
import ctypes as C

import torch

from . import _lib as L

DT = {"f32": L.DC_F32, "fp32": L.DC_F32, "float32": L.DC_F32, "bf16": L.DC_BF16, "bfloat16": L.DC_BF16,
      "f16": L.DC_F16, "fp16": L.DC_F16, "float16": L.DC_F16}
TORCH_DT = {L.DC_F32: torch.float32, L.DC_BF16: torch.bfloat16, L.DC_F16: torch.float16}
DT_SIZE = {L.DC_F32: 4, L.DC_BF16: 2, L.DC_F16: 2}
FAKE_PTR = 1 << 20


def bke(dt):
    return 128 // DT_SIZE[dt]


def round_up(a, b):
    return (a + b - 1) // b * b


class TRef:
    __slots__ = ("name", "dom", "H", "W", "C", "dt", "ld", "eoff", "base", "nbytes", "first", "last", "off", "ext", "qs", "prod")

    def __init__(self, name, dom, H, W, C, dt, nbytes=0, ext=None):
# ... 78 lines not shown
        cout_out = Cout // 2 if act == L.ACT_GEGLU else Cout
        out = self.tensor(name, dom, Hout, Wout, cout_out, src0.dt if out_dt is None else out_dt)
        f = dict(dtype=src0.dt if wdt is None else wdt, taps=taps, stride=stride, upsample=upsample,
                 n_img=self.n[dom], Hin=Hin, Win=Win, Hout=Hout, Wout=Wout,
                 src0=src0, map0=self._map(src0, dom), C0=src0.C, ld0=src0.ld,
                 src1=src1, map1=self._map(src1, dom), C1=src1.C if src1 is not None else 0,
                 ld1=src1.ld if src1 is not None else 0,
                 W=W, Cout=Cout, tile_n=tile_n, bias=bias,
                 rowvec=rowvec, rowvec_map=self._map(rowvec, dom), rowvec_ld=rowvec.ld if rowvec is not None else 0,
                 act=act, gate=gate, gate_map=self._map(gate, dom), gate_ld=gate.ld if gate is not None else 0,
                 residual=residual, res_map=self._map(residual, dom),
                 res_dtype=residual.dt if residual is not None else 0,
                 res_ld=residual.ld if residual is not None else 0,
                 out=out, out_dtype=out.dt, out_ld=out.ld)
        if up4:
            assert upsample and taps == 9
            f.update(up4=1)
            k_real = 4 * src0.C
        if ln_eps:
            f.update(ln_eps=float(ln_eps))
        if side is not None:
            s2, W2 = side
            assert (s2.H, s2.W) == (Hout, Wout) and s2.dt == src0.dt
            f.update(src2=s2, map2=self._map(s2, dom), W2=W2, C2=s2.C, ld2=s2.ld)
        if gn is not None:
            assert gn[0].dom == dom and gn[0].C == f["C0"] + f["C1"], "GroupNorm affine must live in the conv's domain"
            f.update(gn_scale=gn[0], gn_shift=gn[1], gn_silu=int(gn[2]))
        if src1 is not None:
            assert src1.dt == src0.dt and (src1.H, src1.W) == (src0.H, src0.W)
        qs = None
        if qstats:
            parts = int(L.lib().dc_igemm_qstats_parts(self._probe(**f)))
            if parts > 0:
                qs = TRef(name + ".qs", dom, 1, 1, 1, L.DC_F32, nbytes=round_up(self.n[dom] * parts * (Cout // 4) * 2 * 4, 256))
                f.update(qstats=qs)
                out.qs = (qs, parts)
        M = self.n[dom] * Hout * Wout
        kreal = taps * (src0.C + (src1.C if src1 is not None else 0)) if k_real is None else k_real
        es = DT_SIZE[f["dtype"]]
        nsrc = {"bj": self.n["bj"], "unit": self.n["unit"], "ctx": self.n["ctx"]}
        in_bytes = sum(nsrc.get(t.dom, 1) * t.H * t.W * t.C * DT_SIZE[t.dt] for t in (src0, src1, residual) if t is not None)
        meta = dict(name=name, family=f"igemm_{'f32' if f['dtype'] == L.DC_F32 else 'bf16' if f['dtype'] == L.DC_BF16 else 'f16'}_n{tile_n}",
                    flops=2.0 * M * kreal * Cout, bytes=float(in_bytes + kreal * Cout * es + M * cout_out * DT_SIZE[out.dt]),
                    M=M, N=Cout, K=kreal, taps=taps)
        if side is not None:
            meta["flops"] += 2.0 * M * side[0].C * Cout
            meta["K"] = kreal + side[0].C
            meta["bytes"] += float(nsrc.get(side[0].dom, 1) * side[0].H * side[0].W * side[0].C * DT_SIZE[side[0].dt] + side[0].C * Cout * es)
        self._emit(L.OP_IGEMM, L.IgemmParams, f, [src0, src1, rowvec, gate, residual] + (list(gn[:2]) if gn else []) + ([side[0]] if side else []), [out] + ([qs] if qs else []), meta)
        if qstats and gn is None and (qs is not None or (taps == 9 and stride == 1 and not upsample and Hin == 4 and Win == 4)):
            out.prod = len(self.ops) - 1
        return out

    def _probe(self, x=None, **fields):
        if x is not None:
            fields = dict(dict(dtype=x.dt, taps=9, stride=1, upsample=0, n_img=self.n[x.dom], Hin=x.H, Win=x.W, Hout=x.H, Wout=x.W,
                               src0=x, C0=x.C, ld0=x.ld, W=FAKE_PTR, tile_n=128, out=FAKE_PTR, out_dtype=x.dt, out_ld=fields["Cout"]), **fields)
        return L.IgemmParams(**{k: (FAKE_PTR if isinstance(v, TRef) else v) for k, v in fields.items() if v is not None})

    def pn_capable(self, x, Cout, dom):
        if self.pn_off or Cout % 32:
            return False
        return bool(L.lib().dc_igemm_pn_ok(self._probe(x, Cout=Cout, n_img=self.n[dom], pn_groups=32, pn_eps=1e-5)))

    def pn_claim(self, x, gamma, beta, groups, eps, silu):
        if x is None or x.prod is None or x.base is not x or self.pn_off:
            return None
        idx = x.prod
        kind, cls, f = self.ops[idx]
        if f.get("pn_out") is not None or f["Cout"] % groups:
            return None
        if not L.lib().dc_igemm_pn_ok(self._probe(**f, pn_groups=groups, pn_eps=float(eps))):
            return None
        dom = x.dom
        y = self.tensor(x.name + ".pn", dom, x.H, x.W, x.C, x.dt)
        cnt = self.const(torch.zeros(self.n[dom] * ((f["Cout"] + 127) // 128), dtype=torch.int32, device=self.dev))
        y.first = y.last = idx
        f.update(pn_out=y, pn_gamma=gamma, pn_beta=beta, pn_cnt=cnt, pn_ld=y.ld, pn_groups=groups, pn_silu=int(silu), pn_eps=float(eps))
        self.meta[idx]["bytes"] += float(self.n[dom] * x.H * x.W * x.C * DT_SIZE[x.dt])
        self.meta[idx]["pn"] = True
        x.prod = None
        return y

    def up4_ok(self, src0, Cout):
        H2, W2 = 2 * src0.H, 2 * src0.W
        return bool(L.lib().dc_igemm_up4_ok(self._probe(src0, Cout=Cout, upsample=1, Hin=H2, Win=W2, Hout=H2, Wout=W2, bias=FAKE_PTR, up4=1)))

    def ln_ok(self, src0, Cout, act=L.ACT_NONE):
        cout_out = Cout // 2 if act == L.ACT_GEGLU else Cout
        return bool(L.lib().dc_igemm_ln_ok(self._probe(src0, Cout=Cout, taps=1, act=act, out_ld=cout_out, ln_eps=1e-5)))

    def side_ok(self, src0, s2, Cout, residual=None):
        return bool(L.lib().dc_igemm_side_ok(self._probe(src0, Cout=Cout, n_img=self.n[self._dom(src0, s2, residual)], residual=residual,
                                                         res_dtype=src0.dt, res_ld=Cout, src2=s2, W2=FAKE_PTR, C2=s2.C, ld2=s2.ld)))

    def gn_fusable(self, src0, src1, Cout, tile_n=128, out_dt=None):
        return bool(L.lib().dc_igemm_gn_fusable(self._probe(src0, Cout=Cout, n_img=self.n[self._dom(src0, src1)], src1=src1,
                                                            C1=src1.C if src1 is not None else 0, ld1=src1.ld if src1 is not None else 0,
                                                            tile_n=tile_n, out_dtype=src0.dt if out_dt is None else out_dt)))

    def gn_ws_ok(self, x, Cout):
        p = self._probe(x, Cout=Cout, gn_scale=FAKE_PTR, gn_shift=FAKE_PTR, gn_silu=1)
        return L.lib().dc_igemm_variant(p).decode().startswith("conv3_ws")

    def groupnorm_stats(self, name, x0, gamma, beta, groups, eps, x1=None):
        dom = self._dom(x0, x1)
        Cc = x0.C + (x1.C if x1 is not None else 0)
        assert x0.ld == x0.C and (x1 is None or x1.ld == x1.C)
        n, HW = self.n[dom], x0.H * x0.W
        sc = self.tensor(name + ".scale", dom, 1, 1, Cc, L.DC_F32)
        sh = self.tensor(name + ".shift", dom, 1, 1, Cc, L.DC_F32)
        splits = L.lib().dc_groupnorm_splits(n, HW, Cc)
        ws = TRef(name + ".ws", dom, 1, 1, 1, L.DC_F32, nbytes=round_up(L.lib().dc_groupnorm_ws_floats(n, groups, splits) * 4, 256))
        f = dict(x=x0, map0=self._map(x0, dom), x1=x1, map1=self._map(x1, dom), y=None, dtype=x0.dt, out_dtype=x0.dt,
                 n=n, HW=HW, C=x0.C, C1=x1.C if x1 is not None else 0, groups=groups, silu=0, splits=splits, eps=eps,
                 gamma=gamma, beta=beta, ws=ws, out_scale=sc, out_shift=sh)
        qs = None
        if self.qstats_ok(x0, x1, groups, dom):
            qs = x0.qs[0]
            f.update(qstats=qs, qparts=x0.qs[1])
        self._emit(L.OP_GROUPNORM, L.GroupnormParams, f, [x0, x1, qs], [sc, sh, ws],
                   dict(name=name, family="groupnorm_stats", flops=0.0, bytes=(0.0 if qs is not None else 1.0 * n * HW * Cc * DT_SIZE[x0.dt])))
        return sc, sh

    @staticmethod
    def qstats_ok(x0, x1, groups, dom):
        return x1 is None and x0.qs is not None and ((x0.C // groups) % 4 == 0) and x0.dom == dom

    def groupnorm(self, name, x0, gamma, beta, groups, eps, silu, x1=None):
        dom = self._dom(x0, x1)
        Cc = x0.C + (x1.C if x1 is not None else 0)
        assert x0.ld == x0.C and (x1 is None or x1.ld == x1.C)
        out = self.tensor(name, dom, x0.H, x0.W, Cc, x0.dt)
        n, HW = self.n[dom], x0.H * x0.W
        splits = L.lib().dc_groupnorm_splits(n, HW, Cc)
        ws_floats = L.lib().dc_groupnorm_ws_floats(n, groups, splits)
        ws = TRef(name + ".ws", dom, 1, 1, 1, L.DC_F32, nbytes=round_up(ws_floats * 4, 256))
        f = dict(x=x0, map0=self._map(x0, dom), x1=x1, map1=self._map(x1, dom), y=out, dtype=x0.dt, out_dtype=x0.dt,
                 n=n, HW=HW, C=x0.C, C1=x1.C if x1 is not None else 0, groups=groups, silu=int(silu),
                 splits=splits, eps=eps, gamma=gamma, beta=beta, ws=ws)
        qs = None
        if self.qstats_ok(x0, x1, groups, dom):
            qs = x0.qs[0]
            f.update(qstats=qs, qparts=x0.qs[1])
        self._emit(L.OP_GROUPNORM, L.GroupnormParams, f, [x0, x1, qs], [out, ws],
                   dict(name=name, family="groupnorm", flops=0.0, bytes=2.0 * n * HW * Cc * DT_SIZE[x0.dt]))
        return out

    def layernorm(self, name, x, gamma, beta, eps, scale=None, shift=None):
        assert x.ld == x.C
        assert scale is None or x.dom == "unit" or scale.dom == x.dom, "LayerNorm input must already be per-unit"
        out = self.tensor(name, x.dom, x.H, x.W, x.C, x.dt)
        f = dict(x=x, y=out, dtype=x.dt, out_dtype=x.dt, rows=self.n[x.dom] * x.H * x.W, C=x.C,
                 rows_per_sample=x.H * x.W, mod_ld=scale.ld if scale is not None else 0, eps=eps,
                 gamma=gamma, beta=beta, scale=scale, shift=shift, mod_map=self._map(scale, x.dom))
        self._emit(L.OP_LAYERNORM, L.LayernormParams, f, [x, scale, shift], [out],
                   dict(name=name, family="layernorm", flops=0.0, bytes=2.0 * f["rows"] * x.C * DT_SIZE[x.dt]))
        return out

    def attention(self, name, q, k, v, heads, d):
        out = self.tensor(name, q.dom, q.H, q.W, q.C, q.dt)
        dp = q.C // heads
        assert d <= dp and dp * heads == q.C, (d, dp, heads, q.C)
        f = dict(q=q, k=k, v=v, out=out, dtype=q.dt, n=self.n[q.dom], L=q.H * q.W, heads=heads, d=dp,
                 ld_qkv=q.ld, ld_out=out.ld, scale=float(d) ** -0.5)
        Lq = q.H * q.W
# ... 57 lines not shown
        return out

    def eps_mse(self, pred, eps, x_ptr, alpha, sigma, bj_of_unit, img_of_bj, out_index, out_ptr, Cin, v_param, patch=0):
        g = patch if patch > 1 else 1
        f = dict(pred=pred, eps=eps, x=x_ptr, alpha=alpha, sigma=sigma, bj_of_unit=bj_of_unit, img_of_bj=img_of_bj,
                 out_index=out_index, out=out_ptr, n_units=self.n["unit"], C=Cin, H=pred.H * g, W=pred.W * g, ld=pred.ld,
                 v_param=int(v_param), patch=int(patch))
        self._emit(L.OP_EPS_MSE, L.EpsMseParams, f, [pred, eps, alpha, sigma], [],
                   dict(name="eps_mse", family="eps_mse", flops=0.0, bytes=8.0 * self.n["unit"] * Cin * pred.H * g * pred.W * g))

    def err_map(self, pred, eps, x_ptr, alpha, sigma, bj_of_unit, img_of_bj, out_index, acc_ptr, bad_ptr, Cin, v_param, T, cells, patch=0):
        g = patch if patch > 1 else 1
        f = dict(pred=pred, eps=eps, x=x_ptr, alpha=alpha, sigma=sigma, bj_of_unit=bj_of_unit, img_of_bj=img_of_bj,
                 out_index=out_index, acc=acc_ptr, bad=bad_ptr, n_units=self.n["unit"], C=Cin, H=pred.H * g, W=pred.W * g, ld=pred.ld,
                 v_param=int(v_param), patch=int(patch), T=int(T), cells=int(cells))
        self._emit(L.OP_ERR_MAP, L.ErrMapParams, f, [pred, eps, alpha, sigma], [],
                   dict(name="err_map", family="err_map", flops=0.0, bytes=(8.0 * Cin + 8.0) * self.n["unit"] * pred.H * g * pred.W * g))

    def finalize(self, keep_alive=()):
        nops = len(self.ops)
        for t in keep_alive:
            t.base.last = nops
        for i, (kind, _, f) in enumerate(self.ops):
            if kind == L.OP_IGEMM and f.get("pn_out") is not None and isinstance(f.get("out"), TRef):
                b = f["out"].base
                if b.ext is None and b.first == i and b.last == i:
                    self.meta[i]["bytes"] -= float(self.n[b.dom] * b.H * b.W * b.C * DT_SIZE[b.dt])
                    f["out"] = None
        bases = {}
        for _, _, f in self.ops:
            for v in f.values():
                if isinstance(v, TRef) and v.base.ext is None:
                    bases[id(v.base)] = v.base
        order = sorted(bases.values(), key=lambda b: b.first)
        by_last = {}
        for b in order:
            by_last.setdefault(b.last, []).append(b)
        free, top = [], 0
        pending = iter(order)
        nxt = next(pending, None)
        for idx in range(nops + 1):
            while nxt is not None and nxt.first == idx:
                need = nxt.nbytes
                best = None
                for i, (o, s) in enumerate(free):
                    if s >= need and (best is None or s < free[best][1]):
                        best = i
                if best is not None:
                    o, s = free.pop(best)
                    nxt.off = o
                    if s > need:
                        free.append((o + need, s - need))
                else:
                    nxt.off = top
                    top += need
                nxt = next(pending, None)
            for b in by_last.get(idx, []):
                free.append((b.off, b.nbytes))
                free.sort()
                merged = []
                for o, s in free:
                    if merged and merged[-1][0] + merged[-1][1] == o:
                        merged[-1] = (merged[-1][0], merged[-1][1] + s)
                    else:
                        merged.append((o, s))
                free = merged
        self.arena_bytes = top
        self.arena = torch.empty(max(top, 256), dtype=torch.uint8, device=self.dev)
        base_ptr = self.arena.data_ptr()
        assert base_ptr % 256 == 0

        def ptr(v):
            if v is None:
                return None
            if isinstance(v, TRef):
                b = v.base
                p0 = b.ext.data_ptr() if b.ext is not None else base_ptr + b.off
                return p0 + v.eoff * DT_SIZE[v.dt]
            return v

        self.structs = []
        arr = (L.Op * nops)()
        for i, (kind, cls, f) in enumerate(self.ops):
            s = cls()
            for name, ctype in cls._fields_:
                if name not in f:
                    continue
                v = f[name]
                if ctype is L.vp:
                    setattr(s, name, ptr(v))
                else:
                    setattr(s, name, v)
            self.structs.append(s)
            if kind == L.OP_IGEMM:
                self.meta[i]["family"] = L.lib().dc_igemm_variant(s).decode()
            elif kind == L.OP_ATTENTION:
                self.meta[i]["variant"] = L.lib().dc_attention_variant(s).decode()
            elif kind == L.OP_CROSS_ATTENTION:
                self.meta[i]["variant"] = L.lib().dc_cross_attention_variant(s).decode()
            elif kind == L.OP_CROSS_ATTENTION_LEN:
                self.meta[i]["variant"] = L.lib().dc_cross_attention_len_variant(s).decode()
            elif kind == L.OP_GROUPNORM:
                self.meta[i]["variant"] = L.lib().dc_groupnorm_variant(s).decode()
            elif kind == L.OP_LAYERNORM:
                self.meta[i]["variant"] = L.lib().dc_layernorm_variant(s).decode()
            arr[i].kind = kind
            arr[i].params = C.cast(C.pointer(s), C.c_void_p)
        self.op_array = arr
        self.nops = nops
        self.ptr_of = ptr
        return self

    def run(self):
        L.check(L.lib().dc_run_plan(self.op_array, self.nops, L.stream_ptr()), "dc_run_plan")

    def run_timed(self):
        ms = (C.c_float * self.nops)()
        L.check(L.lib().dc_run_plan_timed(self.op_array, self.nops, L.stream_ptr(), ms), "dc_run_plan_timed")
        return list(ms)

    def tensor_view(self, t):
        n = self.n[t.dom]
        assert t.ld == t.C and t.eoff == 0
        if t.base.ext is not None:
            return t.base.ext
        nel = n * t.H * t.W * t.C
        off = t.base.off
        return self.arena[off:off + nel * DT_SIZE[t.dt]].view(TORCH_DT[t.dt]).view(n, t.H, t.W, t.C)


def _dev32(t, device):
    return t.detach().to(device=device, dtype=torch.float32).contiguous()


def _packed(rows, cols, dt, device, lead=()):
    return torch.empty(tuple(lead) + (rows, cols), dtype=TORCH_DT[dt], device=device)


def pack_matrix(w2d, dt, device, tile_n=128, kpad=None, col_scale=None):
    w = _dev32(w2d.reshape(w2d.shape[0], -1), device)
    cout, K = w.shape
    kp = K if kpad is None else kpad
    out = _packed(L.lib().dc_igemm_cout_pad(cout, tile_n), kp, dt, device)
    cs = None if col_scale is None else _dev32(col_scale, device)
    L.check(L.lib().dc_pack_weights_matrix(w.data_ptr(), cout, K, kp, None, None if cs is None else cs.data_ptr(), out.data_ptr(), dt, tile_n,
                                           L.stream_ptr()), "dc_pack_weights_matrix")
    return out


def pack_conv3x3(w, dt, device, tile_n=128, kpad=None, c_lo=0, c_hi=None):
    wd = _dev32(w, device)
    cout, cin = wd.shape[0], wd.shape[1]
    c_hi = cin if c_hi is None else c_hi
    kp = 9 * (c_hi - c_lo) if kpad is None else kpad
    out = _packed(L.lib().dc_igemm_cout_pad(cout, tile_n), kp, dt, device)
    L.check(L.lib().dc_pack_weights_conv3x3(wd.data_ptr(), cout, cin, c_lo, c_hi, kp, out.data_ptr(), dt, tile_n, L.stream_ptr()),
            "dc_pack_weights_conv3x3")
    return out


def pack_up4(w, dt, device, tile_n=128):
    wd = _dev32(w, device)
    cout, cin = wd.shape[0], wd.shape[1]
    out = _packed(L.lib().dc_igemm_cout_pad(cout, tile_n), 4 * cin, dt, device, lead=(4,))
    L.check(L.lib().dc_pack_weights_up4(wd.data_ptr(), cout, cin, out.data_ptr(), dt, tile_n, L.stream_ptr()), "dc_pack_weights_up4")
    return out


def pack_geglu(w, b, dt, device, ln_gamma=None, ln_beta=None):
    wd, bd = _dev32(w, device), _dev32(b, device)
    cout, K = wd.shape
    out = _packed(L.lib().dc_igemm_cout_pad(cout, 128), K, dt, device)
    ob = torch.empty(cout, dtype=torch.float32, device=device)
    ws = torch.empty(cout, dtype=torch.int32, device=device)
    g = None if ln_gamma is None else _dev32(ln_gamma, device)
    be = None if ln_beta is None else _dev32(ln_beta, device)
    L.check(L.lib().dc_pack_weights_geglu(wd.data_ptr(), bd.data_ptr(), cout // 2, K, None if g is None else g.data_ptr(),
                                          None if be is None else be.data_ptr(), out.data_ptr(), ob.data_ptr(), ws.data_ptr(), dt,
                                          L.stream_ptr()), "dc_pack_weights_geglu")
    return out, ob


def fold_layernorm_bias(w, bias, ln_beta, device):
    wd, be = _dev32(w, device), _dev32(ln_beta, device)
    bd = None if bias is None else _dev32(bias, device)
    out = torch.empty(wd.shape[0], dtype=torch.float32, device=device)
    L.check(L.lib().dc_fold_layernorm_bias(wd.data_ptr(), None if bd is None else bd.data_ptr(), be.data_ptr(), wd.shape[0], wd.shape[1],
                                           out.data_ptr(), L.stream_ptr()), "dc_fold_layernorm_bias")
    return out


def geglu_perm(n_half):
    assert n_half % 16 == 0
    idx = []
    for b in range(n_half // 16):
        idx += list(range(16 * b, 16 * b + 16))
        idx += list(range(n_half + 16 * b, n_half + 16 * b + 16))
    return torch.tensor(idx, dtype=torch.long)


def f32c(t, device):
    return t.detach().to(device=device, dtype=torch.float32).contiguous()


def pad_vec(v, rows):
    if v.shape[0] == rows:
        return v
    out = torch.zeros(rows, dtype=v.dtype, device=v.device)
    out[: v.shape[0]] = v
    return out


HEAD_DIMS = (16, 32, 64, 96, 128)


def padded_head_dim(d):
    for dp in HEAD_DIMS:
        if dp >= d:
            return dp
    raise NotImplementedError(f"attention head width {d} is not supported (at most {HEAD_DIMS[-1]})")


def pad_head_rows(w, d, dp):
    if dp == d:
        return w
    x = w.reshape((-1, d) + tuple(w.shape[1:]))
    out = w.new_zeros((x.shape[0], dp) + tuple(w.shape[1:]))
    out[:, :d] = x
    return out.reshape((-1,) + tuple(w.shape[1:]))


def pad_head_cols(w, d, dp):
    if dp == d:
        return w
    x = w.reshape(w.shape[0], -1, d)
    out = w.new_zeros(w.shape[0], x.shape[1], dp)
    out[..., :d] = x
    return out.reshape(w.shape[0], -1)


class UNetWeights:

    def __init__(self, model, dt, device):
        self.dt, self.dev = dt, device
        cfg = model.config
        self.kin = round_up(9 * cfg.in_channels, bke(dt))
        P = {}
        sd = {k: v for k, v in model.state_dict().items()}
# ... 73 lines not shown
            P[key + ".conv1.wa"] = pack_conv3x3(w, self.dt, self.dev, c_lo=0, c_hi=C0)
            P[key + ".conv1.wb"] = pack_conv3x3(w, self.dt, self.dev, c_lo=C0)
        return self.split_shortcut(key, C0)

    def split_shortcut(self, key, C0):
        P, sd = self.P, self._sd
        if key + ".conv_shortcut.weight" in sd and key + ".conv_shortcut.wa" not in P:
            ws = sd[key + ".conv_shortcut.weight"]
            ws = ws.reshape(ws.shape[0], -1)
            P[key + ".conv_shortcut.wa"] = pack_matrix(ws[:, :C0], self.dt, self.dev)
            P[key + ".conv_shortcut.wb"] = pack_matrix(ws[:, C0:], self.dt, self.dev)
        return P

    def fold_layernorms(self, tb_):
        P, sd = self.P, self._sd
        if tb_ + ".qkv.wf" in P:
            return P
        d = sd[tb_ + ".norm1.weight"].shape[0] // self.heads
        qkv = pad_head_rows(torch.cat([sd[tb_ + f".attn1.to_{n}.weight"] for n in "qkv"], 0).float(), d, padded_head_dim(d))
        P[tb_ + ".qkv.wf"] = pack_matrix(qkv, self.dt, self.dev, col_scale=sd[tb_ + ".norm1.weight"])
        P[tb_ + ".qkv.bf"] = fold_layernorm_bias(qkv, None, sd[tb_ + ".norm1.bias"], self.dev)
        P[tb_ + ".ff.net.0.proj.wf"], P[tb_ + ".ff.net.0.proj.bf"] = pack_geglu(
            sd[tb_ + ".ff.net.0.proj.weight"], sd[tb_ + ".ff.net.0.proj.bias"], self.dt, self.dev,
            ln_gamma=sd[tb_ + ".norm3.weight"], ln_beta=sd[tb_ + ".norm3.bias"])
        return P

    def pack_cross(self, fold_ln):
        P, sd = self.P, self._sd
        if "attn2kv.w" not in P:
            kv, self.ckv_off, o = [], {}, 0
            for key in self.attns:
                tb_ = key + ".transformer_blocks.0"
                d = sd[key + ".proj_in.weight"].shape[0] // self.heads
                dp = padded_head_dim(d)
                P[tb_ + ".norm2.g"], P[tb_ + ".norm2.b"] = f32c(sd[tb_ + ".norm2.weight"], self.dev), f32c(sd[tb_ + ".norm2.bias"], self.dev)
                P[tb_ + ".attn2.to_q.w"] = pack_matrix(pad_head_rows(sd[tb_ + ".attn2.to_q.weight"], d, dp), self.dt, self.dev)
                P[tb_ + ".attn2.to_out.0.wc"] = pack_matrix(pad_head_cols(sd[tb_ + ".attn2.to_out.0.weight"], d, dp), self.dt, self.dev)
                P[tb_ + ".attn2.to_out.0.bc"] = f32c(sd[tb_ + ".attn2.to_out.0.bias"], self.dev)
                kv += [pad_head_rows(sd[tb_ + ".attn2.to_k.weight"], d, dp), pad_head_rows(sd[tb_ + ".attn2.to_v.weight"], d, dp)]
                self.ckv_off[key] = o
                o += 2 * self.heads * dp
            self.ckv_total = o
            P["attn2kv.w"] = pack_matrix(torch.cat(kv, 0), L.DC_F32, self.dev)
        if fold_ln:
            for key in self.attns:
                tb_ = key + ".transformer_blocks.0"
                if tb_ + ".attn2.to_q.wf" not in P:
                    d = sd[key + ".proj_in.weight"].shape[0] // self.heads
                    wq = pad_head_rows(sd[tb_ + ".attn2.to_q.weight"].float(), d, padded_head_dim(d))
                    P[tb_ + ".attn2.to_q.wf"] = pack_matrix(wq, self.dt, self.dev, col_scale=sd[tb_ + ".norm2.weight"])
                    P[tb_ + ".attn2.to_q.bf"] = fold_layernorm_bias(wq, None, sd[tb_ + ".norm2.bias"], self.dev)
        return P

    def fold_proj_out(self, key):
        P, sd = self.P, self._sd
        if key + ".ffpo.w" not in P:
            tb_ = key + ".transformer_blocks.0"
            w2, b2 = sd[tb_ + ".ff.net.2.weight"].double(), sd[tb_ + ".ff.net.2.bias"].double()
            wpo = sd[key + ".proj_out.weight"].double()
            wpo = wpo.reshape(wpo.shape[0], -1)
            P[key + ".ffpo.w"] = pack_matrix(torch.cat([wpo @ w2, wpo], 1).float(), self.dt, self.dev)
            P[key + ".ffpo.b"] = f32c((sd[key + ".proj_out.bias"].double() + wpo @ b2).float(), self.dev)
        return P

    def nbytes(self):
        return sum(t.numel() * t.element_size() for t in self.P.values())


class UNetPlan:

    def __init__(self, model, weights, n_bj, n_cls, n_ctx, *, share_trunk=True, score=None, device=None, S=1, varlen=False):
        import os
        assert S >= 1, S
        if varlen and S == 1:
            raise L.DcamdError("a varlen plan needs prompts of S > 1 tokens: one token is always attended")
        fuse_gn_out = os.environ.get("DCAMD_NO_GN_OUT_FUSION") is None
        split_skips = os.environ.get("DCAMD_NO_SKIP_SPLIT") is None
        fold_short = os.environ.get("DCAMD_NO_SHORT_FOLD") is None
        use_qs = os.environ.get("DCAMD_NO_QSTATS") is None
        use_up4 = os.environ.get("DCAMD_NO_UP4") is None
        fold_ln = os.environ.get("DCAMD_NO_LN_FOLD") is None
        fuse_tb = os.environ.get("DCAMD_NO_TBLOCK") is None
        fold_po = os.environ.get("DCAMD_NO_PO_FOLD") is None
        fuse_ws = os.environ.get("DCAMD_NO_GN_WS") is None and use_qs
        cfg = model.config
        dev = device or weights.dev
        dt = weights.dt
        self.dt, self.n_bj, self.n_cls, self.n_ctx, self.S, self.varlen = dt, n_bj, n_cls, n_ctx, S, bool(varlen)
        U = n_bj * n_cls
        pb = PlanBuilder(dev, n_bj, n_cls, n_ctx)
        self.pb = pb
        P = weights.P
        H = W = cfg.sample_size
        C0 = cfg.block_out_channels[0]
        G, eps = cfg.norm_num_groups, cfg.norm_eps
        heads = cfg.attention_head_dim
        i32 = dict(dtype=torch.int32, device=dev)
        f32 = dict(dtype=torch.float32, device=dev)
        self.lam = score["lam"] if score is not None and "lam" in score else torch.zeros(n_bj, **f32)
        self.ctx = torch.zeros((n_ctx, cfg.encoder_hid_dim) if S == 1 else (n_ctx, S, cfg.encoder_hid_dim), **f32)
        self.bj_of_unit = (torch.arange(U, **i32) // n_cls).contiguous()
        if score is not None and "ctx_of_unit" in score:
            self.ctx_of_unit = score["ctx_of_unit"]
        else:
            self.ctx_of_unit = (torch.arange(U, **i32) % n_ctx).contiguous()
        pb.set_map("bj", "unit", self.bj_of_unit)
        pb.set_map("ctx", "unit", self.ctx_of_unit)
        lam = pb.external("lam", self.lam, "bj", 1, 1, 1, L.DC_F32)
        pb.external("ctx", self.ctx, "ctx", 1, S, cfg.encoder_hid_dim, L.DC_F32)
        self.ctx_len = torch.full((n_ctx,), S, **i32) if varlen else None
        ctx_len = pb.const(self.ctx_len)
        kin = weights.kin
        if score is not None:
            self.score = score
            eps_t = pb.external("eps", score["eps"], "bj", 1, 1, 1, L.DC_F32)
            al = pb.external("alpha", score["alpha"], "bj", 1, 1, 1, L.DC_F32)
            sg = pb.external("sigma", score["sigma"], "bj", 1, 1, 1, L.DC_F32)
            a0 = pb.qsample("a0", pb.const(score["x"]), eps_t, al, sg, pb.const(score["img_of_bj"]),
                            cfg.in_channels, H, W, kin, dt, im2col=True)
        else:
            self.a0_buf = torch.zeros(n_bj, H, W, kin, dtype=TORCH_DT[dt], device=dev)
            a0 = pb.external("a0", self.a0_buf, "bj", H, W, kin, dt)
        te = pb.sinusoid("temb.sin", lam, C0, cfg.flip_sin_to_cos, cfg.freq_shift)
        te = pb.igemm("temb.l1", te, pb.const(P["time_embedding.linear_1.w"]), 4 * C0,
                      bias=pb.const(P["time_embedding.linear_1.b"]), act=L.ACT_SILU)
        te = pb.igemm("temb.l2", te, pb.const(P["time_embedding.linear_2.w"]), 4 * C0,
                      bias=pb.const(P["time_embedding.linear_2.b"]), act=L.ACT_SILU)
        tproj = pb.igemm("tproj", te, pb.const(P["tproj.w"]), weights.tproj_total, bias=pb.const(P["tproj.b"]))
        pc = self.ctx_pb = PlanBuilder(dev, 1, 1, n_ctx)
        cctx = pc.external("ctx", self.ctx, "ctx", 1, S, cfg.encoder_hid_dim, L.DC_F32)
        hp = pc.igemm("ctx.hid_proj", cctx, pc.const(P["encoder_hid_proj.w"]), cfg.cross_attention_dim,
                      bias=pc.const(P["encoder_hid_proj.b"]))
        cvec, ckv = {}, {}
        if S == 1:
            vall = pc.igemm("ctx.to_v", hp, pc.const(P["attn2v.w"]), weights.cv_total)
            cv_t = {}
            for k in weights.attns:
                tbk = k + ".transformer_blocks.0"
                Ck = P[k + ".norm.g"].shape[0]
                cv_t[k] = pc.igemm(k + ".cvec", vall.view(weights.cv_off[k], Ck), pc.const(P[tbk + ".attn2.to_out.0.w"]), Ck,
                                   bias=pc.const(P[tbk + ".attn2.to_out.0.b"]))
            pc.finalize(keep_alive=list(cv_t.values()))
            cvec = {k: pb.external(k + ".cvec", pc.tensor_view(t).view(n_ctx, -1), "ctx", 1, 1, t.C, L.DC_F32) for k, t in cv_t.items()}
        else:
            weights.pack_cross(fold_ln)
            kvall = pc.igemm("ctx.to_kv", hp, pc.const(P["attn2kv.w"]), weights.ckv_total, out_dt=dt)
            pc.finalize(keep_alive=[kvall])
            kvx = pb.external("ctx.kv", pc.tensor_view(kvall), "ctx", 1, S, weights.ckv_total, dt)
            for k in weights.attns:
                Cq = heads * padded_head_dim(P[k + ".norm.g"].shape[0] // heads)
                ckv[k] = (kvx.view(weights.ckv_off[k], Cq), kvx.view(weights.ckv_off[k] + Cq, Cq))

        def gn_conv3(gname, cname, x, gamma, beta, groups, Wp, Cout, **kw):
            dom = pb._dom(x, kw.get("rowvec"), kw.get("residual"), kw["side"][0] if kw.get("side") else None)
            y = pb.pn_claim(x, gamma, beta, groups, eps, True)
            if y is not None:
                return pb.igemm(cname, y, Wp, Cout, taps=9, **kw)
            chain = kw.get("qstats") and pb.pn_capable(x, Cout, dom)
            if not chain and fuse_ws and dom == x.dom and pb.qstats_ok(x, None, groups, dom) and pb.gn_ws_ok(x, Cout):
                aff = pb.groupnorm_stats(gname, x, gamma, beta, groups, eps)
                return pb.igemm(cname, x, Wp, Cout, taps=9, gn=(aff[0], aff[1], True), **kw)
            y = pb.groupnorm(gname, x, gamma, beta, groups, eps, True)
            return pb.igemm(cname, y, Wp, Cout, taps=9, **kw)

        def resnet(key, x0, x1=None):
            Cout = P[key + ".conv1.b"].shape[0]
# ... 54 lines not shown
            if S > 1:
                return transformer_prompt(key, tbk, x, h, Cc, d, Cq)
            if fuse_tb and h.dom == pb._dom(h, cvec[key]) and pb.tblock_front_ok(h, heads):
                assert Cq == Cc, "dc_tblock_front takes unpadded heads only"
                h = pb.tblock_front(tbk + ".front", h, pb.const(P[key + ".proj_in.w"]), pb.const(P[key + ".proj_in.b"]),
                                    pb.const(P[tbk + ".norm1.g"]), pb.const(P[tbk + ".norm1.b"]), pb.const(P[tbk + ".qkv.w"]),
                                    pb.const(P[tbk + ".attn1.to_out.0.w"]), pb.const(P[tbk + ".attn1.to_out.0.b"]), cvec[key], heads, 1e-5)
                return transformer_back(key, tbk, x, h, Cc)
            h = pb.igemm(key + ".proj_in", h, pb.const(P[key + ".proj_in.w"]), Cc, bias=pb.const(P[key + ".proj_in.b"]))
            hn = pb.layernorm(tbk + ".ln1", h, pb.const(P[tbk + ".norm1.g"]), pb.const(P[tbk + ".norm1.b"]), 1e-5)
            qkv = pb.igemm(tbk + ".qkv", hn, pb.const(P[tbk + ".qkv.w"]), 3 * Cq)
            o = pb.attention(tbk + ".attn1", qkv.view(0, Cq), qkv.view(Cq, Cq), qkv.view(2 * Cq, Cq), heads, d)
            h = pb.igemm(tbk + ".attn_out", o, pb.const(P[tbk + ".attn1.to_out.0.w"]), Cc,
                         bias=pb.const(P[tbk + ".attn1.to_out.0.b"]), rowvec=cvec[key], residual=h)
            return transformer_back(key, tbk, x, h, Cc)

        def transformer_prompt(key, tbk, x, h, Cc, d, Cq):
            h = pb.igemm(key + ".proj_in", h, pb.const(P[key + ".proj_in.w"]), Cc, bias=pb.const(P[key + ".proj_in.b"]))
            hn = pb.layernorm(tbk + ".ln1", h, pb.const(P[tbk + ".norm1.g"]), pb.const(P[tbk + ".norm1.b"]), 1e-5)
            qkv = pb.igemm(tbk + ".qkv", hn, pb.const(P[tbk + ".qkv.w"]), 3 * Cq)
            o = pb.attention(tbk + ".attn1", qkv.view(0, Cq), qkv.view(Cq, Cq), qkv.view(2 * Cq, Cq), heads, d)
            h = pb.igemm(tbk + ".attn_out", o, pb.const(P[tbk + ".attn1.to_out.0.w"]), Cc,
                         bias=pb.const(P[tbk + ".attn1.to_out.0.b"]), residual=h)
            if fold_ln and pb.ln_ok(h, Cq):
                q2 = pb.igemm(tbk + ".attn2.to_q", h, pb.const(P[tbk + ".attn2.to_q.wf"]), Cq, bias=pb.const(P[tbk + ".attn2.to_q.bf"]), ln_eps=1e-5)
            else:
                hn = pb.layernorm(tbk + ".ln2", h, pb.const(P[tbk + ".norm2.g"]), pb.const(P[tbk + ".norm2.b"]), 1e-5)
                q2 = pb.igemm(tbk + ".attn2.to_q", hn, pb.const(P[tbk + ".attn2.to_q.w"]), Cq)
            o2 = pb.cross_attention(tbk + ".attn2", q2, ckv[key][0], ckv[key][1], heads, d, kv_len=ctx_len)
            h = pb.igemm(tbk + ".attn2_out", o2, pb.const(P[tbk + ".attn2.to_out.0.wc"]), Cc,
                         bias=pb.const(P[tbk + ".attn2.to_out.0.bc"]), residual=h)
            return transformer_back(key, tbk, x, h, Cc)

        def transformer_back(key, tbk, x, h, Cc):
            if fold_ln and pb.ln_ok(h, 8 * Cc, L.ACT_GEGLU):
                weights.fold_layernorms(tbk)
                f = pb.igemm(tbk + ".geglu", h, pb.const(P[tbk + ".ff.net.0.proj.wf"]), 8 * Cc,
                             bias=pb.const(P[tbk + ".ff.net.0.proj.bf"]), act=L.ACT_GEGLU, ln_eps=1e-5)
            else:
                hn = pb.layernorm(tbk + ".ln3", h, pb.const(P[tbk + ".norm3.g"]), pb.const(P[tbk + ".norm3.b"]), 1e-5)
                f = pb.igemm(tbk + ".geglu", hn, pb.const(P[tbk + ".ff.net.0.proj.w"]), 8 * Cc,
                             bias=pb.const(P[tbk + ".ff.net.0.proj.b"]), act=L.ACT_GEGLU)
            if fold_po:
                weights.fold_proj_out(key)
                return pb.igemm(key + ".ff_proj_out", f, pb.const(P[key + ".ffpo.w"]), Cc, src1=h, bias=pb.const(P[key + ".ffpo.b"]), residual=x)
            h = pb.igemm(tbk + ".ff_out", f, pb.const(P[tbk + ".ff.net.2.w"]), Cc, bias=pb.const(P[tbk + ".ff.net.2.b"]),
                         residual=h)
            return pb.igemm(key + ".proj_out", h, pb.const(P[key + ".proj_out.w"]), Cc, bias=pb.const(P[key + ".proj_out.b"]),
                            residual=x)

        h = pb.igemm("conv_in", a0, pb.const(P["conv_in.w"]), C0, bias=pb.const(P["conv_in.b"]),
                     dom=None if share_trunk else "unit", k_real=9 * cfg.in_channels)
        skips = [h]
        boc = cfg.block_out_channels
        for i, kind in enumerate(cfg.down_block_types):
            for j in range(cfg.layers_per_block[i]):
                h = resnet(f"down_blocks.{i}.resnets.{j}", h)
                if kind == "CrossAttnDownBlock2D":
                    h = transformer(f"down_blocks.{i}.attentions.{j}", h)
                skips.append(h)
            if i != len(boc) - 1:
                key = f"down_blocks.{i}.downsamplers.0.conv"
                h = pb.igemm(key, h, pb.const(P[key + ".w"]), boc[i], taps=9, stride=2, bias=pb.const(P[key + ".b"]))
                skips.append(h)
        h = resnet("mid_block.resnets.0", h)
        h = transformer("mid_block.attentions.0", h)
        h = resnet("mid_block.resnets.1", h)
        nb = len(boc)
        rlpb = cfg.layers_per_block[::-1]
        for i, kind in enumerate(cfg.up_block_types):
            for j in range(rlpb[i] + 1):
                h = resnet(f"up_blocks.{i}.resnets.{j}", h, skips.pop())
                if kind == "CrossAttnUpBlock2D":
                    h = transformer(f"up_blocks.{i}.attentions.{j}", h)
            if i != nb - 1:
                key = f"up_blocks.{i}.upsamplers.0.conv"
                if use_up4 and pb.up4_ok(h, h.C):
                    if key + ".w4" not in P:
                        P[key + ".w4"] = pack_up4(weights._sd[key + ".weight"], weights.dt, weights.dev)
                    h = pb.igemm(key, h, pb.const(P[key + ".w4"]), h.C, taps=9, upsample=1, bias=pb.const(P[key + ".b"]), qstats=use_qs, up4=True)
                else:
                    h = pb.igemm(key, h, pb.const(P[key + ".w"]), h.C, taps=9, upsample=1, bias=pb.const(P[key + ".b"]), qstats=use_qs)
        tn_out = 32 if cfg.out_channels <= 32 else 128
        hn = pb.pn_claim(h, pb.const(P["conv_norm_out.g"]), pb.const(P["conv_norm_out.b"]), G, eps, True)
        if hn is not None:
            pred = pb.igemm("conv_out", hn, pb.const(P["conv_out.w"]), cfg.out_channels, taps=9, bias=pb.const(P["conv_out.b"]),
                            out_dt=L.DC_F32, tile_n=tn_out)
        elif (fuse_gn_out and pb.qstats_ok(h, None, G, h.dom) and pb.gn_fusable(h, None, cfg.out_channels, tile_n=tn_out, out_dt=L.DC_F32)):
            aff = pb.groupnorm_stats("conv_norm_out", h, pb.const(P["conv_norm_out.g"]), pb.const(P["conv_norm_out.b"]), G, eps)
            pred = pb.igemm("conv_out", h, pb.const(P["conv_out.w"]), cfg.out_channels, taps=9, bias=pb.const(P["conv_out.b"]),
                            out_dt=L.DC_F32, tile_n=tn_out, gn=(aff[0], aff[1], True))
        else:
            h = pb.groupnorm("conv_norm_out", h, pb.const(P["conv_norm_out.g"]), pb.const(P["conv_norm_out.b"]), G, eps, True)
            pred = pb.igemm("conv_out", h, pb.const(P["conv_out.w"]), cfg.out_channels, taps=9, bias=pb.const(P["conv_out.b"]),
                            out_dt=L.DC_F32, tile_n=tn_out)
        if pred.dom != "unit":
            raise L.DcamdError("backbone has no class-conditioned layer: nothing to score per class")
        self.pred = pred
        if score is not None:
            pb.eps_mse(pred, eps_t, pb.const(score["x"]), al, sg, pb.const(self.bj_of_unit), pb.const(score["img_of_bj"]),
                       pb.const(score["out_index"]), pb.const(score["errors"]), cfg.in_channels, score["v_param"])
            if score.get("emap_acc") is not None:
                pb.err_map(pred, eps_t, pb.const(score["x"]), al, sg, pb.const(self.bj_of_unit), pb.const(score["img_of_bj"]),
                           pb.const(score["out_index"]), pb.const(score["emap_acc"]), pb.const(score["emap_bad"]), cfg.in_channels,
                           score["v_param"], score["emap_T"], score["emap_acc"].shape[0] - 1)
        pb.finalize(keep_alive=[pred])

    def run(self):
        self.pb.run()

    def run_ctx(self):
        self.ctx_pb.run()

    def pred_view(self):
        return self.pb.tensor_view(self.pred)

    @property
    def arena_bytes(self):
        return self.pb.arena_bytes
```

include/dcamd.h:

```cpp
#ifndef DCAMD_H
#define DCAMD_H

#include <stddef.h>
#include <stdint.h>

#ifdef __cplusplus
extern "C" {
#endif

#define DC_ABI_VERSION 5

typedef void* dc_stream;

typedef enum { DC_OK = 0, DC_ERR_ARG = -1, DC_ERR_SHAPE = -2, DC_ERR_DTYPE = -3,
               DC_ERR_ALIGN = -4, DC_ERR_LAUNCH = -5, DC_ERR_UNSUPPORTED = -6 } dc_status;

typedef enum { DC_F32 = 0, DC_BF16 = 1, DC_F16 = 2 } dc_dtype;

typedef enum { DC_ACT_NONE = 0, DC_ACT_SILU = 1, DC_ACT_GEGLU = 2, DC_ACT_GELU_TANH = 3 } dc_act;

int dc_abi_version(void);
const char* dc_last_error(void);
const char* dc_arch(void);

typedef struct {
  const float* x; const float* eps; const float* alpha; const float* sigma;
  const int32_t* img_of_bj;
  void* out; int32_t out_dtype;
  int32_t n_bj, C, H, W, ld, im2col;
  int32_t patch;
} dc_qsample_params;
int dc_qsample(const dc_qsample_params* p, dc_stream s);

int dc_philox_normal(float* out, int64_t rows, int64_t row_len, const int64_t* row_ids, uint64_t seed, dc_stream s);

typedef struct { const float* lam; float* out; int32_t n, dim, flip_sin_to_cos; float freq_shift; } dc_sinusoid_params;
int dc_sinusoid(const dc_sinusoid_params* p, dc_stream s);

typedef struct {
  int32_t dtype, taps, stride, upsample;
  int32_t n_img, Hin, Win, Hout, Wout;
  const void* src0; const int32_t* map0; int32_t C0, ld0;
  const void* src1; const int32_t* map1; int32_t C1, ld1;
  const void* W; int32_t Cout, tile_n;
  const float* bias;
  const float* rowvec; const int32_t* rowvec_map; int32_t rowvec_ld, act;
  const float* gate; const int32_t* gate_map; int32_t gate_ld, pad2_;
  const void* residual; const int32_t* res_map; int32_t res_dtype, res_ld;
  void* out; int32_t out_dtype, out_ld;
  const float* gn_scale; const float* gn_shift; int32_t gn_silu, pad3_;
  const void* src2; const int32_t* map2; const void* W2; int32_t C2, ld2;
  float ln_eps;
  int32_t up4;
  float* qstats;
  void* pn_out; const float* pn_gamma; const float* pn_beta; uint32_t* pn_cnt;
  int32_t pn_ld, pn_groups, pn_silu; float pn_eps;
} dc_igemm_params;
int dc_igemm(const dc_igemm_params* p, dc_stream s);
int32_t dc_igemm_cout_pad(int32_t cout, int32_t tile_n);
const char* dc_igemm_variant(const dc_igemm_params* p);
const char* dc_igemm_instance(const dc_igemm_params* p, int32_t* geom);
int32_t dc_igemm_gn_fusable(const dc_igemm_params* p);
int32_t dc_igemm_side_ok(const dc_igemm_params* p);
int32_t dc_igemm_ln_ok(const dc_igemm_params* p);
int32_t dc_igemm_qstats_parts(const dc_igemm_params* p);
int32_t dc_igemm_pn_ok(const dc_igemm_params* p);
int32_t dc_pn_timeouts(void);
int32_t dc_igemm_up4_ok(const dc_igemm_params* p);

int64_t dc_packed_bytes(int32_t cout, int32_t K, int32_t dtype, int32_t tile_n);
int dc_pack_weights_matrix(const float* w, int32_t cout, int32_t K, int32_t kpad, const int32_t* row_perm, const float* col_scale,
                           void* out, int32_t dtype, int32_t tile_n, dc_stream s);
int dc_pack_weights_conv3x3(const float* w, int32_t cout, int32_t cin, int32_t c_lo, int32_t c_hi, int32_t kpad, void* out,
                            int32_t dtype, int32_t tile_n, dc_stream s);
int dc_pack_weights_up4(const float* w, int32_t cout, int32_t cin, void* out, int32_t dtype, int32_t tile_n, dc_stream s);
int dc_pack_weights_geglu(const float* w, const float* bias, int32_t n_half, int32_t K, const float* ln_gamma, const float* ln_beta,
                          void* out_w, float* out_bias, int32_t* perm_ws, int32_t dtype, dc_stream s);
int dc_fold_layernorm_bias(const float* w, const float* bias, const float* ln_beta, int32_t cout, int32_t K, float* out_bias, dc_stream s);

typedef struct {
  const void* x; const int32_t* map0;
  const void* x1; const int32_t* map1;
  void* y; int32_t dtype, out_dtype;
  int32_t n, HW, C, C1, groups, silu, splits; float eps;
  const float* gamma; const float* beta; float* ws;
  float* out_scale; float* out_shift;
  const float* qstats; int32_t qparts, pad_;
} dc_groupnorm_params;
int dc_groupnorm(const dc_groupnorm_params* p, dc_stream s);
const char* dc_groupnorm_variant(const dc_groupnorm_params* p);
int64_t dc_groupnorm_ws_floats(int32_t n, int32_t groups, int32_t splits);
int32_t dc_groupnorm_splits(int32_t n, int32_t HW, int32_t C);
int64_t dc_workspace_bytes_groupnorm(const dc_groupnorm_params* p);
int64_t dc_workspace_bytes_igemm(const dc_igemm_params* p);

typedef struct {
  const void* x; void* y; int32_t dtype, out_dtype;
  int32_t rows, C, rows_per_sample, mod_ld; float eps;
  const float* gamma; const float* beta;
  const float* scale; const float* shift; const int32_t* mod_map;
} dc_layernorm_params;
int dc_layernorm(const dc_layernorm_params* p, dc_stream s);
const char* dc_layernorm_variant(const dc_layernorm_params* p);
int64_t dc_workspace_bytes_layernorm(const dc_layernorm_params* p);

typedef struct {
  const void* q; const void* k; const void* v; void* out;
  int32_t dtype, n, L, heads, d, ld_qkv, ld_out; float scale;
} dc_attention_params;
int dc_attention(const dc_attention_params* p, dc_stream s);
const char* dc_attention_variant(const dc_attention_params* p);
int64_t dc_workspace_bytes_attention(const dc_attention_params* p);

typedef struct {
  const void* q; const void* k; const void* v; void* out;
  int32_t dtype, n, L, heads, d, ld_qkv, ld_out; float scale;
} dc_attention_wide_params;
int dc_attention_wide(const dc_attention_wide_params* p, dc_stream s);
const char* dc_attention_wide_variant(const dc_attention_wide_params* p);

typedef struct { const void* x; void* out; int32_t dtype, n, H, W, C, ld; } dc_im2col_s2_params;
int dc_im2col_s2(const dc_im2col_s2_params* p, dc_stream s);

typedef struct {
  const void* q; const void* k; const void* v; void* out;
  const int32_t* q_map; const int32_t* kv_map;
  int32_t dtype, n, Lq, S, heads, d, ld_q, ld_kv, ld_out; float scale;
} dc_cross_attention_params;
int dc_cross_attention(const dc_cross_attention_params* p, dc_stream s);
const char* dc_cross_attention_variant(const dc_cross_attention_params* p);

typedef struct {
  const void* q; const void* k; const void* v; void* out;
  const int32_t* q_map; const int32_t* kv_map;
  const int32_t* kv_len;
  int32_t dtype, n, Lq, S, heads, d, ld_q, ld_kv, ld_out; float scale;
} dc_cross_attention_len_params;
int dc_cross_attention_len(const dc_cross_attention_len_params* p, dc_stream s);
const char* dc_cross_attention_len_variant(const dc_cross_attention_len_params* p);

#define DC_ATTENTION_BIAS_MAX_L 512
typedef struct {
  const void* q; const void* k; const void* v; void* out;
  const float* bias;
  const int32_t* kv_len;
  int32_t dtype, n, L, heads, d, ld_qkv, ld_out; float scale;
} dc_attention_bias_params;
int dc_attention_bias(const dc_attention_bias_params* p, dc_stream s);
const char* dc_attention_bias_variant(const dc_attention_bias_params* p);

typedef struct {
  const void* x; void* y; const float* weight; const int32_t* row_len;
// ... 58 lines not shown
typedef struct {
  const float* z; const float* pred; const float* noise; float* out;
  int32_t n, C, H, W, ld, patch, v_param;
  float w, alpha_t, sigma_t, alpha_s, c, sd;
  float one_plus_w;
} dc_ddpm_step_params;
int dc_ddpm_step(const dc_ddpm_step_params* p, dc_stream s);

typedef struct {
  const float* z; const float* pred; const float* noise; float* out;
  int32_t n, C, H, W, ld, patch, v_param;
  int32_t noise_div;
  float w, alpha_t, sigma_t, alpha_s, c, sd;
  float one_plus_w;
  int32_t pad_;
} dc_ddpm_step_shared_params;
int dc_ddpm_step_shared(const dc_ddpm_step_shared_params* p, dc_stream s);

typedef struct {
  const float* z; const float* pred; const float* xprev; float* xhat; float* out;
  int32_t n, C, H, W, ld, patch, v_param, clamp, final_pass;
  float w, one_plus_w, alpha_t, sigma_t, k1, k2, k3;
} dc_solver_step_params;
int dc_solver_step(const dc_solver_step_params* p, dc_stream s);

typedef struct {
  const float* z; const float* pred; const float* x_next; float* out;
  int32_t n, C, H, W, ld, patch, v_param;
  float w, one_plus_w, alpha_t, sigma_t, alpha_s, c, sd;
} dc_ddpm_noise_map_params;
int dc_ddpm_noise_map(const dc_ddpm_noise_map_params* p, dc_stream s);

typedef struct {
  const float* a; const float* r; const int32_t* r_of_a; float* out;
  int32_t n, m, C, H, W, pad_;
} dc_abs_diff_map_params;
int dc_abs_diff_map(const dc_abs_diff_map_params* p, dc_stream s);

int dc_haar_dwt2(const float* in, float* out, int32_t n, int32_t C, int32_t H, int32_t W, float scale, dc_stream s);
int dc_haar_idwt2(const float* in, float* out, int32_t n, int32_t C, int32_t h, int32_t w, float scale, dc_stream s);

int dc_stage_topk(const float* errors, int32_t BS, int32_t C, int32_t T, int32_t t_end, int32_t k, int32_t* keep, float* means, dc_stream s);
int dc_reduce_argmin(const float* errors, int32_t BS, int32_t C, int32_t T, int32_t t_end, int64_t* labels, float* means, dc_stream s);
int dc_stage_maps(const int32_t* keep, int32_t BS, int32_t C, int32_t T, int32_t k, int32_t t0, int32_t n_pairs, int32_t rank,
                  int32_t world, int32_t n_bj, int32_t n_mb, int32_t dump, int32_t* maps, dc_stream s);

int dc_stage_maps_rows(const int32_t* keep, const int32_t* rows, int32_t n_rows, int32_t BS, int32_t C, int32_t T, int32_t k, int32_t t0,
                       int32_t n_pairs, int32_t rank, int32_t world, int32_t n_bj, int32_t n_mb, int32_t dump, int32_t* maps, dc_stream s);
int dc_stage_stop(const float* errors, int32_t BS, int32_t C, int32_t T, int32_t t_end, float z_stop, int32_t* t_done, int64_t* labels,
                  int32_t* active_ids, int32_t* n_active, float* margin_z, dc_stream s);

typedef struct {
  const float* errors;
  float* probs;
  float* entropy; float* margin; float* margin_z;
  int32_t* winner; int32_t* runner; int32_t* invalid;
  float* means; float* delta; int32_t* n_eval;
  int32_t BS, C, T, t_end; float temperature; int32_t pad_;
} dc_class_posterior_params;
int dc_class_posterior(const dc_class_posterior_params* p, dc_stream s);

#define DC_EVIDENCE_FRAC_BITS 30
#define DC_EVIDENCE_VMAX 16384.0f
typedef struct {
  const float* pred; const float* eps; const float* x; const float* alpha; const float* sigma;
  const int32_t* bj_of_unit; const int32_t* img_of_bj; const int32_t* out_index;
  int64_t* acc; int32_t* bad;
  int32_t n_units, C, H, W, ld, v_param, patch;
  int32_t T, cells, pad_;
} dc_err_map_params;
int dc_err_map(const dc_err_map_params* p, dc_stream s);

typedef struct {
  const int64_t* acc; const int32_t* bad; const int32_t* stage_ends; const int32_t* n_eval; const int32_t* winner;
  float* mean_map; float* delta_map; int32_t* invalid;
  int32_t n_stages, BS, C, HW;
} dc_evidence_maps_params;
int dc_evidence_maps(const dc_evidence_maps_params* p, dc_stream s);

typedef enum { DC_OP_QSAMPLE = 1, DC_OP_SINUSOID = 2, DC_OP_IGEMM = 3, DC_OP_GROUPNORM = 4,
               DC_OP_LAYERNORM = 5, DC_OP_ATTENTION = 6, DC_OP_EPS_MSE = 7, DC_OP_TBLOCK_FRONT = 8,
               DC_OP_CROSS_ATTENTION = 9, DC_OP_CROSS_ATTENTION_LEN = 10, DC_OP_ATTENTION_BIAS = 11, DC_OP_RMSNORM = 12,
               DC_OP_EMBED_ROWS = 13, DC_OP_RELU = 14, DC_OP_ATTENTION_CAUSAL = 15, DC_OP_LAYERNORM_ROWS = 16, DC_OP_EMBED_ROWS_POS = 17,
               DC_OP_ACT_PASS = 18, DC_OP_ERR_MAP = 19, DC_OP_ATTENTION_WIDE = 20, DC_OP_IM2COL_S2 = 21 } dc_op_kind;
typedef struct { int32_t kind; int32_t pad_; const void* params; } dc_op;
int dc_run_plan(const dc_op* ops, int32_t n, dc_stream s);
int dc_run_plan_timed(const dc_op* ops, int32_t n, dc_stream s, float* ms);

#ifdef __cplusplus
}
#endif
#endif
```

Measured before the change: 239.1 images/s.

## Fold final GroupNorm+SiLU+conv_out into the last conv3 producer kernel

```diff
diff --git a/diffusion-classifier_amd/_lib.py b/diffusion-classifier_amd/_lib.py
--- a/diffusion-classifier_amd/_lib.py
+++ b/diffusion-classifier_amd/_lib.py
@@ -19,6 +19,7 @@
 EVIDENCE_FRAC_BITS, EVIDENCE_VMAX = 30, 16384.0
 OP_ATTENTION_WIDE, OP_IM2COL_S2 = 20, 21
 ATTENTION_WIDE_DIMS = (256, 512)
+OP_CONV3_PN_TAIL = 22
 
 i32, i64, u64, f32, vp = C.c_int32, C.c_int64, C.c_uint64, C.c_float, C.c_void_p
 
@@ -51,6 +52,15 @@
                 ("pn_ld", i32), ("pn_groups", i32), ("pn_silu", i32), ("pn_eps", f32)]
 
 
+class PnTailParams(C.Structure):
+    _fields_ = [("Wt", vp), ("bias", vp), ("pred", vp), ("ring", vp), ("gamma", vp), ("beta", vp), ("cnt", vp),
+                ("Co", i32), ("pred_ld", i32), ("groups", i32), ("silu", i32), ("eps", f32), ("pad_", i32)]
+
+
+class Conv3PnTailOp(C.Structure):
+    _fields_ = [("conv", C.POINTER(IgemmParams)), ("tail", C.POINTER(PnTailParams))]
+
+
 class GroupnormParams(C.Structure):
     _fields_ = [("x", vp), ("map0", vp), ("x1", vp), ("map1", vp),
                 ("y", vp), ("dtype", i32), ("out_dtype", i32),
@@ -196,7 +206,7 @@
 
 
 EXPORTS = ["dc_abi_version", "dc_last_error", "dc_arch", "dc_qsample", "dc_philox_normal", "dc_sinusoid",
-           "dc_igemm", "dc_igemm_cout_pad", "dc_igemm_variant", "dc_igemm_instance", "dc_igemm_gn_fusable", "dc_igemm_side_ok", "dc_igemm_ln_ok", "dc_igemm_qstats_parts", "dc_igemm_up4_ok", "dc_igemm_pn_ok", "dc_pn_timeouts", "dc_groupnorm", "dc_groupnorm_variant", "dc_groupnorm_ws_floats", "dc_groupnorm_splits",
+           "dc_igemm", "dc_igemm_cout_pad", "dc_igemm_variant", "dc_igemm_instance", "dc_igemm_gn_fusable", "dc_igemm_side_ok", "dc_igemm_ln_ok", "dc_igemm_qstats_parts", "dc_igemm_up4_ok", "dc_igemm_pn_ok", "dc_pn_timeouts", "dc_conv3_pn_tail", "dc_conv3_pn_tail_ok", "dc_conv3_pn_tail_variant", "dc_conv3_pn_tail_ring_floats", "dc_groupnorm", "dc_groupnorm_variant", "dc_groupnorm_ws_floats", "dc_groupnorm_splits",
            "dc_layernorm", "dc_layernorm_variant", "dc_attention", "dc_attention_variant", "dc_attention_wide", "dc_attention_wide_variant", "dc_im2col_s2", "dc_cross_attention", "dc_cross_attention_variant", "dc_cross_attention_len", "dc_cross_attention_len_variant", "dc_attention_bias", "dc_attention_bias_variant", "dc_rmsnorm", "dc_embed_rows", "dc_relu", "dc_attention_causal", "dc_attention_causal_variant", "dc_layernorm_rows", "dc_embed_rows_pos", "dc_act_pass", "dc_tblock_front", "dc_tblock_front_ok", "dc_eps_mse", "dc_err_map", "dc_evidence_maps", "dc_ddpm_step", "dc_ddpm_step_shared", "dc_solver_step", "dc_ddpm_noise_map", "dc_abs_diff_map", "dc_haar_dwt2", "dc_haar_idwt2", "dc_stage_topk", "dc_reduce_argmin", "dc_stage_maps", "dc_stage_maps_rows", "dc_stage_stop", "dc_class_posterior", "dc_run_plan", "dc_run_plan_timed",
            "dc_packed_bytes", "dc_pack_weights_matrix", "dc_pack_weights_conv3x3", "dc_pack_weights_up4", "dc_pack_weights_geglu",
            "dc_fold_layernorm_bias", "dc_workspace_bytes_groupnorm", "dc_workspace_bytes_igemm", "dc_workspace_bytes_attention",
@@ -279,6 +289,14 @@
     L.dc_tblock_front_ok.restype = C.c_int32
     L.dc_pn_timeouts.argtypes = []
     L.dc_pn_timeouts.restype = C.c_int32
+    L.dc_conv3_pn_tail.argtypes = [C.POINTER(IgemmParams), C.POINTER(PnTailParams), vp]
+    L.dc_conv3_pn_tail.restype = i32
+    L.dc_conv3_pn_tail_ok.argtypes = [C.POINTER(IgemmParams), C.POINTER(PnTailParams)]
+    L.dc_conv3_pn_tail_ok.restype = i32
+    L.dc_conv3_pn_tail_variant.argtypes = [C.POINTER(IgemmParams), C.POINTER(PnTailParams)]
+    L.dc_conv3_pn_tail_variant.restype = C.c_char_p
+    L.dc_conv3_pn_tail_ring_floats.argtypes = [C.POINTER(IgemmParams), C.POINTER(PnTailParams)]
+    L.dc_conv3_pn_tail_ring_floats.restype = i64
     L.dc_igemm_side_ok.argtypes = [C.POINTER(IgemmParams)]
     L.dc_igemm_side_ok.restype = C.c_int32
     L.dc_igemm_variant.argtypes = [C.POINTER(IgemmParams)]
diff --git a/diffusion-classifier_amd/csrc/api.hip b/diffusion-classifier_amd/csrc/api.hip
--- a/diffusion-classifier_amd/csrc/api.hip
+++ b/diffusion-classifier_amd/csrc/api.hip
@@ -79,6 +79,11 @@
       case DC_OP_EPS_MSE: rc = dc_eps_mse(static_cast<const dc_eps_mse_params*>(ops[i].params), s); break;
       case DC_OP_ERR_MAP: rc = dc_err_map(static_cast<const dc_err_map_params*>(ops[i].params), s); break;
       case DC_OP_ATTENTION_WIDE: rc = dc_attention_wide(static_cast<const dc_attention_wide_params*>(ops[i].params), s); break;
+      case DC_OP_CONV3_PN_TAIL: {
+        const dc_conv3_pn_tail_op* t = static_cast<const dc_conv3_pn_tail_op*>(ops[i].params);
+        rc = dc_conv3_pn_tail(t->conv, t->tail, s);
+        break;
+      }
       case DC_OP_IM2COL_S2: rc = dc_im2col_s2(static_cast<const dc_im2col_s2_params*>(ops[i].params), s); break;
       default: dc_set_error("dc_run_plan: op %d has unknown kind %d", i, ops[i].kind); return DC_ERR_ARG;
     }
diff --git a/diffusion-classifier_amd/csrc/conv3_halo.h b/diffusion-classifier_amd/csrc/conv3_halo.h
--- a/diffusion-classifier_amd/csrc/conv3_halo.h
+++ b/diffusion-classifier_amd/csrc/conv3_halo.h
@@ -72,3 +72,17 @@
 #ifndef HALO_XDEPTH
 #define HALO_XDEPTH 3
 #endif
+
+struct PnTail {
+  const void* Wt;
+  const float* bias;
+  float* pred;
+  float* ring;
+  int Co, pred_ld;
+};
+#define PN_TAIL_RING(tw, th) (2 * ((tw) + 2) + 2 * (th))
+__host__ __device__ __forceinline__ int pn_tail_ring_slot(int oy, int ox, int tw, int th) {
+  if (oy < 0) return ox + 1;
+  if (oy >= th) return tw + 2 + ox + 1;
+  return 2 * (tw + 2) + (ox < 0 ? 0 : th) + oy;
+}
diff --git a/diffusion-classifier_amd/csrc/conv3_halo.hip b/diffusion-classifier_amd/csrc/conv3_halo.hip
--- a/diffusion-classifier_amd/csrc/conv3_halo.hip
+++ b/diffusion-classifier_amd/csrc/conv3_halo.hip
@@ -19,8 +19,10 @@
 #include "conv3_halo_plan.h"
 DC_CLOCK_DECL(conv3_halo)
 
-template <typename T, int NW, int NTAP = 9, int MODE = 0, bool STG = false, bool PN = false>
-__global__ __launch_bounds__(NW * 64, 2) void conv3_halo_kernel(const IgemmArgs a, const HaloGeom g) {
+template <typename T, int NW, int NTAP = 9, int MODE = 0, bool STG = false, bool PN = false, typename... TL>
+__global__ __launch_bounds__(NW * 64, 2) void conv3_halo_kernel(const IgemmArgs a, const HaloGeom g, const TL... tl) {
+  constexpr bool TAIL = sizeof...(TL) == 1;
+  static_assert(sizeof...(TL) <= 1 && (!TAIL || (PN && NW == 4 && NTAP == 9 && MODE == 1 && sizeof(T) == 2)), "tail fold: the 16-bit 4-wave exchange form");
   static_assert(!PN || (MODE == 1 && NW == 4 && !STG) || ((MODE == 0 || MODE == 2) && NW == 8 && STG && NTAP == 9), "producer-side GroupNorm: one-image-per-patch forms, or 8x8 / 4x4 images");
   constexpr bool PNX = PN && NW == 4, PNL = PN && NW == 8;
   static_assert(!STG || NW == 8, "staggered loop: the 8-wave kernel");
@@ -486,6 +488,13 @@
     pc.scr = reinterpret_cast<float2*>(pc.tiles > 1 ? smem + wave * 4096 : smem + wn * 256);
     pc.flag = reinterpret_cast<int*>(brv + 384);
     pc.eps = a.pn_eps; pc.silu = a.pn_silu;
+    if constexpr (TAIL) {
+      PnTailCtx tc;
+      tc.p = [](const PnTail& p, auto...) { return p; }(tl...);
+      tc.zs = reinterpret_cast<float*>(smem);
+      tc.wm = wm; tc.ltw = g.ltw; tc.lth = g.lth; tc.tx = tx; tc.ty = ty; tc.tiles_x = g.tiles_x; tc.lpt = g.lpt; tc.H = g.H; tc.W = g.W;
+      epi_halo_pn<T>(a, acc, tile_n, wn, lq, rowfn, brv + wn * 64 + lq * 8, pc, tc);
+    } else
     epi_halo_pn<T>(a, acc, tile_n, wn, lq, rowfn, brv + wn * 64 + lq * 8, pc);
   } else if constexpr (STAGE_BRV) {
     epi_direct_act<T, TM, DC_ACT_NONE, false, true>(a, acc, tile_n, wn, lq, nw0, nw1, rowfn, EpiNoPre(), qsfn, HaloLdsBias{brv + wn * 64 + lq * 8});
@@ -780,6 +789,34 @@
   return dc_check_launch("dc_igemm(conv3_halo)");
 }
 
+template <typename T>
+static int launch_tail(const HaloPlan& pl, const IgemmArgs& a, const PnTail& tl, hipStream_t s) {
+  static bool attr_done = false;
+  void (*kern)(const IgemmArgs, const HaloGeom, const PnTail) = conv3_halo_kernel<T, 4, 9, 1, false, true, PnTail>;
+  if (!attr_done) {
+    (void)hipFuncSetAttribute(reinterpret_cast<const void*>(kern), hipFuncAttributeMaxDynamicSharedMemorySize, HaloCfg<4>::LDS);
+    attr_done = true;
+  }
+  hipLaunchKernelGGL(kern, dim3(pl.grid), dim3(256), HaloCfg<4>::LDS, s, a, pl.g, tl);
+  return dc_check_launch("dc_conv3_pn_tail(conv3_halo)");
+}
+
+static_assert(2 * 256 * PN_TAIL_ZLD * 4 <= 2 * HaloCfg<4>::XBUF + HaloCfg<4>::WR * HALO_WST, "tail fold: the z image must fit the halo buffers and the W ring");
+
+bool dc_conv3_halo_tail_ok(const IgemmArgs& a, const HaloPlan& pl, int dtype, int Co) {
+  const HaloKey& k = pl.key;
+  return pl.status == DC_OK && k.NW == 4 && k.NTAP == 9 && k.MODE == 1 && !k.STG && k.PN && (dtype == DC_BF16 || dtype == DC_F16) &&
+         a.Cout == 128 && a.tiles_n == 1 && Co >= 1 && 9 * Co <= 32 && Co <= 3 && !a.out;
+}
+
+int dc_conv3_halo_tail_launch(const HaloPlan& pl, const IgemmArgs& a0, int dtype, const PnTail& tl, hipStream_t s) {
+  if (pl.status != DC_OK) { dc_set_error("%s", pl.message); return pl.status; }
+  if (!dc_conv3_halo_tail_ok(a0, pl, dtype, tl.Co)) { dc_set_error("dc_conv3_pn_tail: no tail instance for this problem"); return DC_ERR_UNSUPPORTED; }
+  IgemmArgs a = a0;
+  a.tiles_m = pl.tiles_m;
+  return dtype == DC_BF16 ? launch_tail<__bf16>(pl, a, tl, s) : launch_tail<_Float16>(pl, a, tl, s);
+}
+
 constexpr int PN_MAX_TILES = 16;
 bool dc_conv3_halo_pn_ok(const IgemmArgs& a, const HaloPlan& pl, bool up4) {
   static const bool off = getenv("DCAMD_NO_PN") != nullptr;
diff --git a/diffusion-classifier_amd/csrc/conv3_halo_plan.h b/diffusion-classifier_amd/csrc/conv3_halo_plan.h
--- a/diffusion-classifier_amd/csrc/conv3_halo_plan.h
+++ b/diffusion-classifier_amd/csrc/conv3_halo_plan.h
@@ -67,4 +67,8 @@
 int dc_conv3_halo_launch(const HaloPlan& pl, const IgemmArgs& a, int dtype, bool up4, hipStream_t s);
 bool dc_conv3_halo_pn_ok(const IgemmArgs& a, const HaloPlan& pl, bool up4);
 HaloPlan dc_conv3_thin_plan(const IgemmArgs& a, int n_img);
+bool dc_conv3_halo_tail_ok(const IgemmArgs& a, const HaloPlan& pl, int dtype, int Co);
+int dc_conv3_halo_tail_launch(const HaloPlan& pl, const IgemmArgs& a, int dtype, const PnTail& tl, hipStream_t s);
+int dc_pn_tail_combine_launch(float* pred, const float* ring, int n_img, int ltw, int lth, int tiles_x, int tiles_y, int H, int W, int Co, int ld,
+                              hipStream_t s);
 HaloPlan dc_conv3_ws_plan(const IgemmArgs& a, int n_img);
diff --git a/diffusion-classifier_amd/csrc/elementwise.hip b/diffusion-classifier_amd/csrc/elementwise.hip
--- a/diffusion-classifier_amd/csrc/elementwise.hip
+++ b/diffusion-classifier_amd/csrc/elementwise.hip
@@ -552,3 +552,45 @@
   }
   return dc_check_launch("dc_im2col_s2");
 }
+
+#include "conv3_halo.h"
+__global__ __launch_bounds__(256) void pn_tail_combine_kernel(float* pred, const float* ring, int total, int ltw, int lth, int tiles_x, int tiles_y,
+                                                              int H, int W, int Co, int ld) {
+  const int idx = blockIdx.x * 256 + threadIdx.x;
+  if (idx >= total) return;
+  const int tw = 1 << ltw, th = 1 << lth, tiles = tiles_x * tiles_y;
+  const int nb = 2 * tw + 2 * (th - 2);
+  const int b = idx % nb, rest = idx / nb, tile = rest % tiles, n = rest / tiles;
+  const int ty = tile / tiles_x, tx = tile - ty * tiles_x;
+  int py, px;
+  if (b < 2 * tw) { py = b < tw ? 0 : th - 1; px = b & (tw - 1); }
+  else { const int c = b - 2 * tw; py = 1 + (c >> 1); px = (c & 1) ? tw - 1 : 0; }
+  const int gy = ty * th + py, gx = tx * tw + px;
+  float s[3] = {0.f, 0.f, 0.f};
+  float* o = pred + ((size_t)n * H * W + (size_t)gy * W + gx) * ld;
+  bool any = false;
+  for (int dy = -1; dy <= 1; ++dy)
+    for (int dx = -1; dx <= 1; ++dx) {
+      if (!dy && !dx) continue;
+      const int ny = ty + dy, nx = tx + dx;
+      if ((unsigned)ny >= (unsigned)tiles_y || (unsigned)nx >= (unsigned)tiles_x) continue;
+      const int oy = gy - ny * th, ox = gx - nx * tw;
+      if (oy < -1 || oy > th || ox < -1 || ox > tw) continue;
+      const float* r = ring + (((size_t)n * tiles + ny * tiles_x + nx) * PN_TAIL_RING(tw, th) + pn_tail_ring_slot(oy, ox, tw, th)) * Co;
+      if (!any) { for (int co = 0; co < 3; ++co) if (co < Co) s[co] = o[co]; any = true; }
+      for (int co = 0; co < 3; ++co) if (co < Co) s[co] += r[co];
+    }
+  if (any)
+    for (int co = 0; co < 3; ++co) if (co < Co) o[co] = s[co];
+}
+
+int dc_pn_tail_combine_launch(float* pred, const float* ring, int n_img, int ltw, int lth, int tiles_x, int tiles_y, int H, int W, int Co, int ld,
+                              hipStream_t s) {
+  if (tiles_x * tiles_y == 1) return DC_OK;
+  const int tw = 1 << ltw, th = 1 << lth;
+  const long long total = (long long)n_img * tiles_x * tiles_y * (2 * tw + 2 * (th - 2));
+  if (total <= 0 || total > 0x7fffffffLL) { dc_set_error("dc_conv3_pn_tail: bad combine extent %lld", total); return DC_ERR_SHAPE; }
+  hipLaunchKernelGGL(pn_tail_combine_kernel, dim3((unsigned)((total + 255) / 256)), dim3(256), 0, s, pred, ring, (int)total, ltw, lth, tiles_x, tiles_y,
+                     H, W, Co, ld);
+  return dc_check_launch("dc_conv3_pn_tail(combine)");
+}
diff --git a/diffusion-classifier_amd/csrc/epi_pn.h b/diffusion-classifier_amd/csrc/epi_pn.h
--- a/diffusion-classifier_amd/csrc/epi_pn.h
+++ b/diffusion-classifier_amd/csrc/epi_pn.h
@@ -1,5 +1,6 @@
 #pragma once
 #include "igemm_epilogue.h"
+#include "conv3_halo.h"
 
 #ifndef PN_TIMEOUT_TICKS
 #define PN_TIMEOUT_TICKS 3000000ull
@@ -20,6 +21,49 @@
   float eps;
   int silu;
 };
+
+#define PN_TAIL_ZLD 36
+struct PnNoTail { static constexpr bool on = false; };
+struct PnTailCtx {
+  static constexpr bool on = true;
+  PnTail p;
+  float* zs;
+  int wm, ltw, lth, tx, ty, tiles_x, lpt, H, W;
+};
+__device__ __forceinline__ void pn_tail_finish(const PnTailCtx& t, int sample) {
+  const int tw = 1 << t.ltw, th = 1 << t.lth, hw = tw + 2, npos = (th + 2) * hw;
+  const int Co = t.p.Co;
+  const int tile = t.ty * t.tiles_x + t.tx;
+  for (int pos = threadIdx.x; pos < npos; pos += 256) {
+    const int hy = pos / hw, hx = pos - hy * hw;
+    const int oy = hy - 1, ox = hx - 1;
+    const int gy = (t.ty << t.lth) + oy, gx = (t.tx << t.ltw) + ox;
+    if ((unsigned)gy >= (unsigned)t.H || (unsigned)gx >= (unsigned)t.W) continue;
+    float s[3] = {0.f, 0.f, 0.f};
+#pragma unroll
+    for (int tap = 0; tap < 9; ++tap) {
+      const int py = oy + tap / 3 - 1, px = ox + tap % 3 - 1;
+      if ((unsigned)py < (unsigned)th && (unsigned)px < (unsigned)tw) {
+        const float* z0 = t.zs + ((py << t.ltw) + px) * PN_TAIL_ZLD + tap * Co;
+        const float* z1 = z0 + 256 * PN_TAIL_ZLD;
+#pragma unroll
+        for (int co = 0; co < 3; ++co)
+          if (co < Co) s[co] += z0[co] + z1[co];
+      }
+    }
+    if ((unsigned)oy < (unsigned)th && (unsigned)ox < (unsigned)tw) {
+      float* o = t.p.pred + ((size_t)sample * t.H * t.W + (size_t)gy * t.W + gx) * t.p.pred_ld;
+#pragma unroll
+      for (int co = 0; co < 3; ++co)
+        if (co < Co) o[co] = s[co] + (t.p.bias ? t.p.bias[co] : 0.f);
+    } else {
+      float* o = t.p.ring + ((((size_t)sample << t.lpt) + tile) * PN_TAIL_RING(tw, th) + pn_tail_ring_slot(oy, ox, tw, th)) * Co;
+#pragma unroll
+      for (int co = 0; co < 3; ++co)
+        if (co < Co) o[co] = s[co];
+    }
+  }
+}
 
 __device__ __forceinline__ void pn_fold_row(const float2* scr, int parts, int q0, int qpg, int lr, float nq, float& mean, float& var) {
 #pragma clang fp contract(off)
@@ -45,9 +89,9 @@
   var = fmaxf(m2 / (R * nq), 0.f);
 }
 
-template <typename T, typename RowFn>
+template <typename T, typename RowFn, typename TL = PnNoTail>
 __device__ __forceinline__ void epi_halo_pn(const IgemmArgs& a, f32x4 (&acc)[4][8], int tile_n, int wn, int lq, RowFn rowfn,
-                                            const float* brv, const PnCtx& c) {
+                                            const float* brv, const PnCtx& c, const TL& tl = TL()) {
   constexpr int TM = 8, NK = 2;
   constexpr bool res16 = sizeof(T) == 2;
   const int abl = DC_HALO_ABL();
@@ -227,6 +271,14 @@
   }
   __builtin_amdgcn_s_waitcnt(0xC07F);
   __builtin_amdgcn_wave_barrier();
+  chunk16 wt[2][NK];
+  if constexpr (TL::on) {
+#pragma unroll
+    for (int mf = 0; mf < 2; ++mf)
+#pragma unroll
+      for (int k = 0; k < NK; ++k)
+        wt[mf][k] = *reinterpret_cast<const chunk16*>(reinterpret_cast<const T*>(tl.p.Wt) + (mf * 16 + lrp) * 128 + wn * 64 + 32 * k + lq * 8);
+  }
   float ga[NK][8], gb[NK][8];
   {
     const float nq = 512.0f;
@@ -259,6 +311,44 @@
     }
   }
   DC_STAMP(6);
+  if constexpr (TL::on) {
+    f32x4 z[2][TM];
+    auto tail_mma = [&](auto actc) {
+      constexpr bool ACT = decltype(actc)::value;
+#pragma unroll
+      for (int j = 0; j < TM; ++j) {
+        chunk16 y[NK];
+#pragma unroll
+        for (int k = 0; k < NK; ++k) {
+          float v[8];
+#pragma unroll
+          for (int e = 0; e < 8; ++e) {
+            float x = acc[2 * k + (e >> 2)][j][e & 3] * ga[k][e] + gb[k][e];
+            if (ACT) x = silu_t<T>(x);
+            v[e] = x;
+          }
+          y[k] = f_to_chunk<T>(v);
+        }
+#pragma unroll
+        for (int mf = 0; mf < 2; ++mf) {
+          z[mf][j] = f32x4{0.f, 0.f, 0.f, 0.f};
+#pragma unroll
+          for (int k = 0; k < NK; ++k) z[mf][j] = Mma<T>::run(wt[mf][k], y[k], z[mf][j]);
+        }
+      }
+    };
+    if (c.silu && !(abl & 32)) tail_mma(EpiIC<1>{});
+    else tail_mma(EpiIC<0>{});
+    __syncthreads();
+#pragma unroll
+    for (int j = 0; j < TM; ++j)
+#pragma unroll
+      for (int mf = 0; mf < 2; ++mf)
+        *reinterpret_cast<f32x4*>(tl.zs + (wn * 256 + tl.wm * 128 + j * 16 + lrp) * PN_TAIL_ZLD + mf * 16 + 4 * lq) = z[mf][j];
+    __syncthreads();
+    pn_tail_finish(tl, c.sample);
+    return;
+  }
   auto store_norm = [&](auto actc) {
     constexpr bool ACT = decltype(actc)::value;
 #pragma unroll
diff --git a/diffusion-classifier_amd/csrc/igemm.hip b/diffusion-classifier_amd/csrc/igemm.hip
--- a/diffusion-classifier_amd/csrc/igemm.hip
+++ b/diffusion-classifier_amd/csrc/igemm.hip
@@ -397,6 +397,64 @@
 
 extern "C" int32_t dc_pn_timeouts(void) { return (int32_t)dc_conv3_halo_pn_timeouts(); }
 
+struct TailChoice { IgemmArgs a; IgemmChoice c; int status = DC_OK; const char* tag = nullptr; const char* message = nullptr; };
+
+static TailChoice tail_choose(const dc_igemm_params* conv, const dc_pn_tail_params* tail, bool probe) {
+  TailChoice t;
+  auto fail = [&](int st, const char* tag, const char* msg) -> TailChoice& { t.status = st; t.tag = tag; t.message = msg; return t; };
+  if (!conv || !tail) return fail(DC_ERR_ARG, "invalid", "dc_conv3_pn_tail: null params");
+  if (conv->out || conv->pn_out) return fail(DC_ERR_UNSUPPORTED, "tail-raw-output", "dc_conv3_pn_tail: the conv's own output (out / pn_out) is never stored; leave both null");
+  dc_igemm_params q = *conv;
+  q.pn_out = g_probe_dummy;
+  q.pn_gamma = tail->gamma; q.pn_beta = tail->beta; q.pn_cnt = tail->cnt;
+  q.pn_ld = 0; q.pn_groups = tail->groups; q.pn_silu = tail->silu; q.pn_eps = tail->eps;
+  if (probe) {
+    if (!q.qstats) q.qstats = g_probe_dummy;
+    if (!q.pn_gamma) q.pn_gamma = g_probe_dummy;
+    if (!q.pn_beta) q.pn_beta = g_probe_dummy;
+    if (!q.pn_cnt) q.pn_cnt = reinterpret_cast<uint32_t*>(g_probe_dummy);
+    if (!(q.pn_eps > 0.f)) q.pn_eps = 1e-5f;
+  } else if (!tail->Wt || !tail->pred || !tail->ring || ((uintptr_t)tail->Wt & 15) || (((uintptr_t)tail->pred | (uintptr_t)tail->ring | (uintptr_t)tail->bias) & 3)) {
+    return fail(DC_ERR_ARG, "invalid", "dc_conv3_pn_tail: Wt (16-byte aligned), pred and ring must be given");
+  }
+  if (q.pn_groups <= 0) return fail(DC_ERR_ARG, "invalid", "dc_conv3_pn_tail: groups");
+  if (igemm_validate_and_fill(&q, t.a) != DC_OK) return fail(DC_ERR_ARG, "invalid", nullptr);
+  t.c = igemm_choose(&q, t.a);
+  if (t.c.status != DC_OK) return fail(t.c.status, t.c.tag, t.c.message);
+  if (t.c.kernel != IG_HALO || !t.c.pn || !dc_conv3_halo_tail_ok(t.a, t.c.halo, q.dtype, tail->Co) || tail->pred_ld < tail->Co)
+    return fail(DC_ERR_UNSUPPORTED, "tail-unsupported",
+                "dc_conv3_pn_tail: needs a 16-bit 3x3 conv with Cout = 128 on the 4-wave producer-GroupNorm form and 1 <= Co <= 3 (see dc_conv3_pn_tail_ok)");
+  return t;
+}
+
+extern "C" int32_t dc_conv3_pn_tail_ok(const dc_igemm_params* conv, const dc_pn_tail_params* tail) {
+  return tail_choose(conv, tail, true).status == DC_OK ? 1 : 0;
+}
+
+extern "C" const char* dc_conv3_pn_tail_variant(const dc_igemm_params* conv, const dc_pn_tail_params* tail) {
+  const TailChoice t = tail_choose(conv, tail, true);
+  if (t.status != DC_OK) return t.tag;
+  return conv->dtype == DC_BF16 ? "conv3_halo<bf16,4w,pn,tail>" : "conv3_halo<f16,4w,pn,tail>";
+}
+
+extern "C" int64_t dc_conv3_pn_tail_ring_floats(const dc_igemm_params* conv, const dc_pn_tail_params* tail) {
+  const TailChoice t = tail_choose(conv, tail, true);
+  if (t.status != DC_OK) return 0;
+  const HaloGeom& g = t.c.halo.g;
+  return (long long)conv->n_img * g.tiles_x * g.tiles_y * PN_TAIL_RING(1 << g.ltw, 1 << g.lth) * tail->Co;
+}
+
+extern "C" int dc_conv3_pn_tail(const dc_igemm_params* conv, const dc_pn_tail_params* tail, dc_stream stream) {
+  const TailChoice t = tail_choose(conv, tail, false);
+  if (t.status != DC_OK) { if (t.message) dc_set_error("%s", t.message); return t.status; }
+  hipStream_t s = reinterpret_cast<hipStream_t>(stream);
+  const PnTail tl{tail->Wt, tail->bias, tail->pred, tail->ring, tail->Co, tail->pred_ld};
+  const int rc = dc_conv3_halo_tail_launch(t.c.halo, t.a, conv->dtype, tl, s);
+  if (rc != DC_OK) return rc;
+  const HaloGeom& g = t.c.halo.g;
+  return dc_pn_tail_combine_launch(tail->pred, tail->ring, conv->n_img, g.ltw, g.lth, g.tiles_x, g.tiles_y, g.H, g.W, tail->Co, tail->pred_ld, s);
+}
+
 extern "C" int32_t dc_igemm_up4_ok(const dc_igemm_params* p) {
   if (!p) return 0;
   dc_igemm_params q = *p;
diff --git a/diffusion-classifier_amd/engine.py b/diffusion-classifier_amd/engine.py
--- a/diffusion-classifier_amd/engine.py
+++ b/diffusion-classifier_amd/engine.py
@@ -184,6 +184,50 @@
         x.prod = None
         return y
 
+    def pn_tail(self, name, x, gamma, beta, groups, eps, silu, Wt, bias, Co):
+        if x is None or x.prod is None or x.base is not x or self.pn_off:
+            return None
+        idx = x.prod
+        kind, cls, f = self.ops[idx]
+        b = x.base
+        if kind != L.OP_IGEMM or f.get("pn_out") is not None or f["Cout"] % groups or b.ext is not None or b.first != idx or b.last != idx:
+            return None
+        dom = x.dom
+        pred = self.tensor(name, dom, x.H, x.W, Co, L.DC_F32)
+        t = dict(tail_Wt=Wt, tail_bias=bias, tail_pred=pred, tail_Co=Co, tail_pred_ld=pred.ld,
+                 pn_gamma=gamma, pn_beta=beta, pn_groups=groups, pn_silu=int(silu), pn_eps=float(eps))
+        probe = dict(f, out=None, **t)
+        conv_p, tail_p = self._tail_structs(probe, lambda v: FAKE_PTR if isinstance(v, TRef) else v)
+        ring_floats = int(L.lib().dc_conv3_pn_tail_ring_floats(conv_p, tail_p))
+        if ring_floats <= 0 or not L.lib().dc_conv3_pn_tail_ok(conv_p, tail_p):
+            return None
+        t["tail_ring"] = self.const(torch.zeros(ring_floats, dtype=torch.float32, device=self.dev))
+        t["pn_cnt"] = self.const(torch.zeros(self.n[dom], dtype=torch.int32, device=self.dev))
+        f.update(t, out=None)
+        self.ops[idx] = (L.OP_CONV3_PN_TAIL, L.Conv3PnTailOp, f)
+        pred.first = pred.last = idx
+        M = self.n[dom] * x.H * x.W
+        m = self.meta[idx]
+        m.update(kind=L.OP_CONV3_PN_TAIL, tail=True, pn=True)
+        m["flops"] += 2.0 * M * x.C * 9 * Co
+        m["bytes"] += float(-M * x.C * DT_SIZE[x.dt] + M * Co * 4 + 2 * ring_floats * 4 + 32 * x.C * DT_SIZE[x.dt])
+        x.prod = None
+        return pred
+
+    @staticmethod
+    def _tail_structs(f, ptr):
+        conv, tail = L.IgemmParams(), L.PnTailParams()
+        for name, ctype in L.IgemmParams._fields_:
+            if name in f and f[name] is not None and not name.startswith("pn_"):
+                setattr(conv, name, ptr(f[name]) if ctype is L.vp else f[name])
+        src = dict(Wt="tail_Wt", bias="tail_bias", pred="tail_pred", ring="tail_ring", gamma="pn_gamma", beta="pn_beta", cnt="pn_cnt",
+                   Co="tail_Co", pred_ld="tail_pred_ld", groups="pn_groups", silu="pn_silu", eps="pn_eps")
+        for name, ctype in L.PnTailParams._fields_:
+            v = f.get(src.get(name))
+            if v is not None:
+                setattr(tail, name, ptr(v) if ctype is L.vp else v)
+        return conv, tail
+
     def up4_ok(self, src0, Cout):
         H2, W2 = 2 * src0.H, 2 * src0.W
         return bool(L.lib().dc_igemm_up4_ok(self._probe(src0, Cout=Cout, upsample=1, Hin=H2, Win=W2, Hout=H2, Wout=W2, bias=FAKE_PTR, up4=1)))
@@ -407,6 +451,14 @@
         self.structs = []
         arr = (L.Op * nops)()
         for i, (kind, cls, f) in enumerate(self.ops):
+            if kind == L.OP_CONV3_PN_TAIL:
+                conv, tail = self._tail_structs(f, ptr)
+                s = cls(C.pointer(conv), C.pointer(tail))
+                self.structs.append((s, conv, tail))
+                self.meta[i]["family"] = L.lib().dc_conv3_pn_tail_variant(conv, tail).decode()
+                arr[i].kind = kind
+                arr[i].params = C.cast(C.pointer(s), C.c_void_p)
+                continue
             s = cls()
             for name, ctype in cls._fields_:
                 if name not in f:
@@ -489,6 +541,15 @@
     cout, cin = wd.shape[0], wd.shape[1]
     out = _packed(L.lib().dc_igemm_cout_pad(cout, tile_n), 4 * cin, dt, device, lead=(4,))
     L.check(L.lib().dc_pack_weights_up4(wd.data_ptr(), cout, cin, out.data_ptr(), dt, tile_n, L.stream_ptr()), "dc_pack_weights_up4")
+    return out
+
+
+def pack_tail(w, dt, device):
+    wd = _dev32(w, device)
+    co, cin = wd.shape[0], wd.shape[1]
+    assert 9 * co <= 32 and cin == 128 and tuple(wd.shape[2:]) == (3, 3), tuple(wd.shape)
+    out = torch.zeros(32, cin, dtype=TORCH_DT[dt], device=device)
+    out[:9 * co] = wd.permute(2, 3, 0, 1).reshape(9 * co, cin).to(TORCH_DT[dt])
     return out
 
 
@@ -728,6 +789,7 @@
         fold_ln = os.environ.get("DCAMD_NO_LN_FOLD") is None
         fuse_tb = os.environ.get("DCAMD_NO_TBLOCK") is None
         fold_po = os.environ.get("DCAMD_NO_PO_FOLD") is None
+        fold_tail = os.environ.get("DCAMD_NO_TAIL_FOLD") is None
         fuse_ws = os.environ.get("DCAMD_NO_GN_WS") is None and use_qs
         cfg = model.config
         dev = device or weights.dev
@@ -948,8 +1010,16 @@
                 else:
                     h = pb.igemm(key, h, pb.const(P[key + ".w"]), h.C, taps=9, upsample=1, bias=pb.const(P[key + ".b"]), qstats=use_qs)
         tn_out = 32 if cfg.out_channels <= 32 else 128
-        hn = pb.pn_claim(h, pb.const(P["conv_norm_out.g"]), pb.const(P["conv_norm_out.b"]), G, eps, True)
-        if hn is not None:
+        pred = None
+        if fold_tail and cfg.out_channels <= 3 and h.C == 128 and dt != L.DC_F32:
+            if "conv_out.wt" not in P:
+                P["conv_out.wt"] = pack_tail(weights._sd["conv_out.weight"], weights.dt, weights.dev)
+            pred = pb.pn_tail("conv_out", h, pb.const(P["conv_norm_out.g"]), pb.const(P["conv_norm_out.b"]), G, eps, True,
+                              pb.const(P["conv_out.wt"]), pb.const(P["conv_out.b"]), cfg.out_channels)
+        hn = None if pred is not None else pb.pn_claim(h, pb.const(P["conv_norm_out.g"]), pb.const(P["conv_norm_out.b"]), G, eps, True)
+        if pred is not None:
+            pass
+        elif hn is not None:
             pred = pb.igemm("conv_out", hn, pb.const(P["conv_out.w"]), cfg.out_channels, taps=9, bias=pb.const(P["conv_out.b"]),
                             out_dt=L.DC_F32, tile_n=tn_out)
         elif (fuse_gn_out and pb.qstats_ok(h, None, G, h.dom) and pb.gn_fusable(h, None, cfg.out_channels, tile_n=tn_out, out_dt=L.DC_F32)):
diff --git a/include/dcamd.h b/include/dcamd.h
--- a/include/dcamd.h
+++ b/include/dcamd.h
@@ -68,6 +68,17 @@
 int32_t dc_pn_timeouts(void);
 int32_t dc_igemm_up4_ok(const dc_igemm_params* p);
 
+typedef struct {
+  const void* Wt; const float* bias; float* pred; float* ring;
+  const float* gamma; const float* beta; uint32_t* cnt;
+  int32_t Co, pred_ld, groups, silu; float eps; int32_t pad_;
+} dc_pn_tail_params;
+int dc_conv3_pn_tail(const dc_igemm_params* conv, const dc_pn_tail_params* tail, dc_stream s);
+int32_t dc_conv3_pn_tail_ok(const dc_igemm_params* conv, const dc_pn_tail_params* tail);
+const char* dc_conv3_pn_tail_variant(const dc_igemm_params* conv, const dc_pn_tail_params* tail);
+int64_t dc_conv3_pn_tail_ring_floats(const dc_igemm_params* conv, const dc_pn_tail_params* tail);
+typedef struct { const dc_igemm_params* conv; const dc_pn_tail_params* tail; } dc_conv3_pn_tail_op;
+
 int64_t dc_packed_bytes(int32_t cout, int32_t K, int32_t dtype, int32_t tile_n);
 int dc_pack_weights_matrix(const float* w, int32_t cout, int32_t K, int32_t kpad, const int32_t* row_perm, const float* col_scale,
                            void* out, int32_t dtype, int32_t tile_n, dc_stream s);
@@ -292,7 +303,8 @@
                DC_OP_LAYERNORM = 5, DC_OP_ATTENTION = 6, DC_OP_EPS_MSE = 7, DC_OP_TBLOCK_FRONT = 8,
                DC_OP_CROSS_ATTENTION = 9, DC_OP_CROSS_ATTENTION_LEN = 10, DC_OP_ATTENTION_BIAS = 11, DC_OP_RMSNORM = 12,
                DC_OP_EMBED_ROWS = 13, DC_OP_RELU = 14, DC_OP_ATTENTION_CAUSAL = 15, DC_OP_LAYERNORM_ROWS = 16, DC_OP_EMBED_ROWS_POS = 17,
-               DC_OP_ACT_PASS = 18, DC_OP_ERR_MAP = 19, DC_OP_ATTENTION_WIDE = 20, DC_OP_IM2COL_S2 = 21 } dc_op_kind;
+               DC_OP_ACT_PASS = 18, DC_OP_ERR_MAP = 19, DC_OP_ATTENTION_WIDE = 20, DC_OP_IM2COL_S2 = 21,
+               DC_OP_CONV3_PN_TAIL = 22  } dc_op_kind;
 typedef struct { int32_t kind; int32_t pad_; const void* params; } dc_op;
 int dc_run_plan(const dc_op* ops, int32_t n, dc_stream s);
 int dc_run_plan_timed(const dc_op* ops, int32_t n, dc_stream s, float* ms);
```

Result: faster. 241.9 images/s (median of 6 runs) (+1.2%).
